# dropbox/rust-brotli

Hardware: AMD Instinct MI355X
Metric: compress MB/s at q5 lgwin22 (higher is better)
Workload: dtype u8; 1 GPU; 64 MiB synthetic English-like text per GPU, quality=5, lgwin=22, one-shot BrotliEncoderCompress (H6), input and stream resident in HBM; input_bytes_total=67108864, compressed_bytes=16370400

## Files before the change

rust-brotli_amd/csrc/device_api.h:

```cpp
#ifndef BROTLI_MI355X_DEVICE_API_H_
#define BROTLI_MI355X_DEVICE_API_H_

#include <stddef.h>
#include <stdint.h>

#include <vector>

#include "lz77_types.h"

#define BR_STREAM (::brotli_mi355x::dev_stream_flushed())

struct ihipStream_t;
namespace brotli_mi355x {

ihipStream_t* dev_stream_flushed();

void* dev_alloc(size_t bytes);
void* dev_alloc_uninit(size_t bytes);
#ifdef BROTLI_HOST_EMU
void dev_free(void* p);
#else
void dev_free(void* p) noexcept;
static_assert(noexcept(dev_free(nullptr)), "blocks are freed in destructors");
#endif
void dev_memset(void* p, int value, size_t bytes);
void dev_h2d(void* dst, const void* src, size_t bytes);
void dev_d2h(void* dst, const void* src, size_t bytes);
void dev_h2d_bulk(void* dst, const void* src, size_t bytes);
void dev_d2h_bulk(void* dst, const void* src, size_t bytes);
void dev_d2h_async(void* dst, const void* src, size_t bytes);
void dev_d2d(void* dst, const void* src, size_t bytes);
void dev_sync();
void dev_mark();
void dev_wait_mark();
void dev_mark_n(int i);
void dev_wait_mark_n(int i);
void* dev_host_alloc(size_t bytes);
void dev_host_free(void* p);
void dev_pool_counters(double* out4, bool reset);
void dev_make_room_for(size_t bytes, size_t own_share);
void dev_make_room(unsigned min_free_share);
size_t dev_trim_pool();
int dev_current_device();
void dev_use_device(int device);
int dev_device_count();
const char* dev_name();

class DevBlocks {
 public:
  DevBlocks() = default;
  DevBlocks(DevBlocks&& o) noexcept : blocks_(std::move(o.blocks_)) { o.blocks_.clear(); }
  DevBlocks& operator=(DevBlocks&& o) noexcept {
    if (this != &o) {
      clear();
      blocks_.swap(o.blocks_);
    }
    return *this;
  }
  ~DevBlocks() { clear(); }
  template <typename T = void>
  T* zeroed(size_t bytes) { return (T*)get(bytes, true); }
  template <typename T = void>
  T* uninit(size_t bytes) { return (T*)get(bytes, false); }
  template <typename T>
  void drop(T*& p) {
    if (p) dev_free(forget(p));
    p = nullptr;
  }
  template <typename T>
  T* give(DevBlocks& to, T*& p) {
    T* q = p;
    to.blocks_.reserve(to.blocks_.size() + 1);
    to.blocks_.push_back(forget(p));
    p = nullptr;
    return q;
  }
  void clear() noexcept {
    for (void* p : blocks_) dev_free(p);
    blocks_.clear();
  }

 private:
  void* get(size_t bytes, bool zero) {
    blocks_.reserve(blocks_.size() + 1);
    blocks_.push_back(zero ? dev_alloc(bytes) : dev_alloc_uninit(bytes));
    return blocks_.back();
  }
  void* forget(const void* p) {
    for (size_t i = blocks_.size(); i-- > 0;)
      if (blocks_[i] == p) {
        void* q = blocks_[i];
        blocks_.erase(blocks_.begin() + (ptrdiff_t)i);
        return q;
      }
    return nullptr;
  }
  std::vector<void*> blocks_;
};

struct DevMem {
  DevBlocks blocks;
  static constexpr size_t kArenaBytes = (size_t)4 << 20, kSmall = (size_t)256 << 10;
  uint8_t* arena = nullptr;
  size_t arena_used = kArenaBytes;
  template <typename T>
  T* alloc(size_t count) {
    const size_t bytes = (count * sizeof(T) + 64 + 255) & ~(size_t)255;
    if (bytes > kSmall) return blocks.zeroed<T>(bytes);
    if (arena_used + bytes > kArenaBytes) {
      arena = blocks.zeroed<uint8_t>(kArenaBytes);
      arena_used = 0;
    }
    T* p = (T*)(arena + arena_used);
    arena_used += bytes;
    return p;
  }
};

struct DeviceTables {
  const uint16_t* dict_hash;
  const uint8_t* dict_data;
  const uint32_t* dict_offsets_by_length;
  const uint8_t* dict_size_bits_by_length;
  const float* logs_16;
  const float* logs_8;
  const uint8_t* utf8_context_lookup;
  const uint8_t* signed_context_lookup;
  const uint16_t* dict_lut_buckets;
  const uint32_t* dict_lut_words;
};
const DeviceTables& dev_tables();

static constexpr uint32_t kChangedCap = 1u << 16;
struct RankInitialHint {
  uint32_t first_block_start, block_bytes;
  uint32_t prefix_is_dictionary;
};
struct SegGeometry;

struct Lz77Buffers {
  uint8_t* text;
  uint16_t* keys;
  uint32_t* by_key;
  uint16_t* sorted_keys;
  uint8_t* fbits;
  uint32_t* info[2];
  uint32_t* sorted[2];
  uint32_t* key_base;
  uint32_t* key_first;
  uint32_t* key_last;
  uint32_t* changed_keys;
  uint32_t* changed_count;
  uint16_t* stag;
  uint32_t* rows;
  void* checkpoints = nullptr;
  uint32_t* rows_changed_lo = nullptr;
  uint32_t* rows_changed_hi = nullptr;
  uint32_t splice_lists = 1;
  uint32_t* dict_items = nullptr;
  uint32_t* changed_slot;
  uint32_t* row_ctl;
  uint32_t* reset_counts;
  const uint32_t* count_base;
  uint32_t* run_end;
  unsigned long long* smask;
  uint32_t* gprev;
  uint8_t* big_tile;
  unsigned long long* pot = nullptr;
  uint32_t* pot_state = nullptr;
  uint32_t* pot_list = nullptr;
  uint32_t pot_list_cap = 0;
  uint32_t* flip_cells = nullptr;
  uint32_t cell_shift = 0, cells_per_key = 0;
  uint32_t changed_cap;
  uint16_t* sorted_tag[2] = {nullptr, nullptr};
  uint32_t* search_log = nullptr;
  uint32_t* recheck_list = nullptr;
  uint32_t* recheck_count = nullptr;
  uint32_t recheck_cap = 0;
  uint8_t* flags[2];
  Command* cmds;
  Segment* segments;
  SegEntry* entries;
  SegExit* exits;
  void* sort_tmp;
  size_t sort_tmp_bytes;
};

size_t lz77_sort_tmp_bytes(uint32_t total_bytes);

void lz77_compute_keys(const Lz77Params& P, const Lz77Buffers& B);
void lz77_run_table(const Lz77Params& P, const Lz77Buffers& B);
void lz77_init_flags(const Lz77Params& P, const Lz77Buffers& B, uint32_t first_block_start, const uint8_t* prefix_flags_host = nullptr,
                     uint32_t prefix_flags_bytes = 0);
void lz77_sort_by_key(const Lz77Params& P, const Lz77Buffers& B);
void lz77_rank_flags(const Lz77Params& P, const Lz77Buffers& B, int which, int rbuf, const RankInitialHint* initial = nullptr);
void lz77_rows_init(const Lz77Params& P, const Lz77Buffers& B, int which, const RankInitialHint* initial, bool has_big_keys);
void lz77_rows_update(const Lz77Params& P, const Lz77Buffers& B, int prev, int next, const SegGeometry& geo, uint8_t* dirty_dev,
                      bool has_big_keys);
void lz77_parse_round(const Lz77Params& P, const Lz77Buffers& B, int which, int rbuf, uint32_t first_segment);
void lz77_parse_list(const Lz77Params& P, const Lz77Buffers& B, int which, int rbuf, const uint32_t* list_dev, uint8_t* sched_dev,
                     uint32_t count);
void lz77_scatter_entries(const Lz77Buffers& B, const uint32_t* index_dev, const SegEntry* entries_dev, uint32_t count);
void lz77_gather_results(const Lz77Buffers& B, const uint32_t* list_dev, uint32_t count, const uint8_t* sched_dev, uint32_t num_segments,
                         SegExit* exits_out, uint32_t* cont_count, uint32_t* cont_index, SegExit* cont_exits, SegEntry* cont_entries);
void lz77_diff_flags(const Lz77Params& P, const Lz77Buffers& B, int prev, int next);
struct BurstBuffers {
  uint8_t* sched = nullptr;
  uint8_t* cand_dirty = nullptr;
  uint8_t* entry_dirty = nullptr;
  uint8_t* touched = nullptr;
  uint8_t* stale = nullptr;
  SegEntry* new_entries = nullptr;
  uint32_t* list = nullptr;
  uint32_t* counters = nullptr;
};
void lz77_chain_check(const Lz77Params& P, const Lz77Buffers& B, const BurstBuffers& U);
void lz77_flags_catch_up(const Lz77Params& P, const Lz77Buffers& B, const BurstBuffers& U, int src, int dst);
void lz77_diff_flags_touched(const Lz77Params& P, const Lz77Buffers& B, const BurstBuffers& U, int prev, int next);
void lz77_reset_rows_changed(const Lz77Params& P, const Lz77Buffers& B);
void lz77_drop_checkpoints(const Lz77Params& P, const Lz77Buffers& B, const uint32_t* list_dev, uint32_t count);
void lz77_burst_count(const Lz77Params& P, const Lz77Buffers& B, const BurstBuffers& U);
void lz77_burst_schedule(const Lz77Params& P, const Lz77Buffers& B, const BurstBuffers& U);
void lz77_gather_touched(const Lz77Params& P, const Lz77Buffers& B, const BurstBuffers& U, uint32_t* index_out, SegExit* exits_out, SegEntry* entries_out);
struct SegGeometry {
  uint32_t prefix_bytes, first_block_start, block_bytes, num_blocks, num_segments, block_size ;
  const uint32_t* block_first_segment;
  const uint32_t* block_segment_bytes;
};
void lz77_validate(const Lz77Params& P, const Lz77Buffers& B, int which, int rbuf_old, int rbuf_new, const SegGeometry& geo,
                   uint8_t* dirty_dev);
void lz77_recheck_searches(const Lz77Params& P, const Lz77Buffers& B, int rbuf, const SegGeometry& geo, uint8_t* dirty_dev);
static constexpr uint32_t kRerankChunk = 4096;
struct RerankChunk {
  uint32_t key_lo;
  uint32_t begin, end;
  uint32_t first_sum;
  uint32_t my_sum;
};
void lz77_rerank_keys(const Lz77Params& P, const Lz77Buffers& B, int which, int rbuf, const RerankChunk* chunks_dev, uint32_t num_chunks,
                      uint32_t* sums_dev, const SegGeometry& geo, uint8_t* dirty_dev);
void lz77_parse_custom(const Lz77Params& P, const Lz77Buffers& B, int which, int rbuf, const Segment* segments_dev,
                       SegEntry* entries_dev, SegExit* exits_dev, uint32_t count);
struct CacheCheck {
  uint32_t segment;
  int32_t cache[4];
};
void lz77_check_cache(const Lz77Params& P, const Lz77Buffers& B, int which, const CacheCheck* items_dev, uint32_t count, uint8_t* ok_dev);
void lz77_key_counts(const Lz77Params& P, const Lz77Buffers& B, int which, uint32_t upto, uint32_t* out_dev, bool with_base = true);
void lz77_parse_timing(double* total_ms, uint32_t* launches, uint64_t* segments, uint64_t* work = nullptr);
void lz77_sample_histograms(const uint8_t* text_dev, const uint32_t* ranges, uint32_t count, uint32_t* out);
void lz77_sample_histogram(const uint8_t* text, uint32_t start, uint32_t bytes, uint32_t* histo256_dev);
void lz77_gather_commands(const Lz77Params& P, const Lz77Buffers& B, uint32_t num_segments, const uint32_t* offsets_dev,
                          const uint32_t* counts_dev, Command* out);

struct ZopfliJob {
  uint32_t quality = 10, lgwin = 22;
  uint32_t use_dictionary = 1;
  uint32_t dist_alphabet_size = 0;
  uint32_t block_bytes = 0;
  uint32_t* buckets = nullptr;
  uint32_t* forest = nullptr;
  void* nodes = nullptr;
  float* literal_costs = nullptr;
  float* cost_dist = nullptr;
  float* cost_cmd = nullptr;
  unsigned long long* matches = nullptr;
  uint32_t* num_matches = nullptr;
  Command* tmp_cmds = nullptr;
  uint32_t* histo = nullptr;
  uint32_t* forest_new = nullptr;
  uint32_t* forest_bak = nullptr;
  uint32_t* buckets_bak = nullptr;
  uint8_t* rerooted = nullptr;
  uint32_t* ctl = nullptr;
};
void lz77_zopfli_init(const ZopfliJob& J);
void lz77_zopfli_import(const ZopfliJob& J, const uint32_t* buckets_src, const uint32_t* forest_src, uint32_t delta);
void lz77_zopfli_prepend(const Lz77Params& P, const Lz77Buffers& B, const ZopfliJob& J, uint32_t dict_bytes);
bool lz77_zopfli_block(const Lz77Params& P, const Lz77Buffers& B, const ZopfliJob& J, uint32_t block);

struct LiveBuffers {
  uint16_t* num = nullptr;
  uint32_t* buckets = nullptr;
  uint32_t* slot_of = nullptr;
  uint32_t* rank[2] = {nullptr, nullptr};
  uint32_t* entry[2] = {nullptr, nullptr};
  uint8_t* changed_key = nullptr;
  LiveBlockState* state = nullptr;
  uint32_t tables = 0;
  uint32_t span_blocks = 1;
};
void lz77_live_slots(const Lz77Params& P, const Lz77Buffers& B, const LiveBuffers& L);
void lz77_live_index(const Lz77Params& P, const Lz77Buffers& B, const LiveBuffers& L, int which);
void lz77_live_materialise(const Lz77Params& P, const Lz77Buffers& B, const LiveBuffers& L, int which, const uint32_t* first_dev,
                           const uint32_t* start_dev, uint32_t count);
void lz77_live_parse(const Lz77Params& P, const Lz77Buffers& B, const LiveBuffers& L, int which, const uint32_t* first_dev, uint32_t count);
void lz77_live_verify(const Lz77Params& P, const Lz77Buffers& B, const LiveBuffers& L, int prev, int next, const SegGeometry& geo,
                      const uint8_t* reparsed_dev, uint8_t* dirty_dev);

void lz77_patch_commands(Command* cmds, const CmdPatch* patches_dev, uint32_t n);

template <typename T>
struct PinnedArray {
  T* ptr = nullptr;
  size_t cap = 0, n = 0;
  PinnedArray() = default;
  PinnedArray(const PinnedArray&) = delete;
  PinnedArray& operator=(const PinnedArray&) = delete;
  ~PinnedArray() { dev_host_free(ptr); }
  void resize_discard(size_t count) {
    if (count > cap) {
      dev_host_free(ptr);
      cap = count + count / 4 + 16;
      ptr = (T*)dev_host_alloc(cap * sizeof(T));
    }
    n = count;
  }
  void assign(size_t count, const T& v) {
    resize_discard(count);
    for (size_t i = 0; i < count; ++i) ptr[i] = v;
  }
  T* data() { return ptr; }
  const T* data() const { return ptr; }
  size_t size() const { return n; }
  T& operator[](size_t i) { return ptr[i]; }
  const T& operator[](size_t i) const { return ptr[i]; }
};

}
#endif
```

rust-brotli_amd/csrc/lz77_kernels.hip:

```cpp
#include <hip/hip_runtime.h>
#include <stdexcept>
#include <string>
#include <utility>
#include <string.h>
#include <mutex>
#include <vector>

#include "device_api.h"
#include "lz77_chain.h"
#include "lz77_rows.h"
#include "lz77_groups.h"
#include "device_scan.h"
#include "lz77_parse_args.h"
#include "zopfli_device.h"
#include "batch_greedy_device.h"

namespace brotli_mi355x {

void hip_check(hipError_t e, const char* what) {
  if (e == hipSuccess) return;
  (void)hipGetLastError();
  throw std::runtime_error(std::string("HIP error in ") + what + ": " + hipGetErrorString(e));
}

static constexpr uint32_t kSortTile = 4096;

__global__ __launch_bounds__(256) void k_compute_keys(const uint8_t* __restrict__ text, uint16_t* __restrict__ keys,
                                                      uint32_t n, uint32_t valid_n, uint32_t kind, uint32_t bucket_bits,
                                                      uint64_t hash_mask, uint32_t* __restrict__ run_samples,
                                                      const uint16_t* __restrict__ dict_hash, uint32_t* __restrict__ dict_items,
                                                      uint32_t num_tiles, uint32_t* __restrict__ hist) {
  __shared__ uint32_t h[256];
  for (uint32_t tile = blockIdx.x; tile < num_tiles; tile += gridDim.x) {
    const uint32_t tile_base = tile * kSortTile;
    const uint32_t tile_n = n - tile_base < kSortTile ? n - tile_base : kSortTile;
    if (hist != nullptr) {
      h[threadIdx.x] = 0;
      __syncthreads();
    }
#pragma unroll 4
    for (uint32_t e = threadIdx.x; e < tile_n; e += 256) {
      const uint32_t i = tile_base + e;
      if (dict_items != nullptr) {
        const uint32_t dh = ((br_load32(text + i) * 0x1e35a7bdu) >> (32 - 14)) << 1;
        dict_items[i] = (uint32_t)dict_hash[dh] | ((uint32_t)dict_hash[dh + 1] << 16);
      }
      uint32_t key = 0xffffu;
      if (i < valid_n) {
        if ((i & 63u) == 0 && i + 16 <= n) {
          const uint64_t v = br_load64(text + i);
          if (v == (v & 0xffull) * 0x0101010101010101ull && br_load64(text + i + 8) == v && *(volatile uint32_t*)run_samples < 4096u)
            atomicAdd(run_samples, 1u);
        }
        if (kind == 6) {
          const uint64_t v = (br_load64(text + i) & hash_mask) * 0x1fe35a7bd3579bd3ull;
          key = (uint32_t)(v >> (64 - bucket_bits));
        } else {
          const uint32_t v = br_load32(text + i) * 0x1e35a7bdu;
          key = v >> (32 - bucket_bits);
        }
      }
      keys[i] = (uint16_t)key;
      if (hist != nullptr) atomicAdd(&h[key & 255u], 1u);
    }
    if (hist != nullptr) {
      __syncthreads();
      hist[threadIdx.x * num_tiles + tile] = h[threadIdx.x];
    }
  }
  if (dict_items != nullptr && blockIdx.x == 0 && threadIdx.x == 0) {
    const uint32_t dh = ((br_load32(text + n) * 0x1e35a7bdu) >> (32 - 14)) << 1;
    dict_items[n] = (uint32_t)dict_hash[dh] | ((uint32_t)dict_hash[dh + 1] << 16);
  }
}

struct SortScratch {
  uint16_t* keys_tmp;
  uint32_t* vals_tmp;
  uint16_t* tags_tmp;
  uint32_t* hist;
  uint32_t* scratch;
};
static SortScratch sort_scratch(const Lz77Buffers& B, uint32_t n) {
  const uint32_t tiles = (n + kSortTile - 1) / kSortTile;
  SortScratch s;
  uint8_t* tmp = (uint8_t*)B.sort_tmp;
  s.keys_tmp = (uint16_t*)tmp;
  tmp += ((size_t)n * 2 + 255) & ~(size_t)255;
  s.vals_tmp = (uint32_t*)tmp;
  tmp += ((size_t)n * 4 + 255) & ~(size_t)255;
  s.tags_tmp = (uint16_t*)tmp;
  tmp += ((size_t)n * 2 + 255) & ~(size_t)255;
  s.hist = (uint32_t*)tmp;
  tmp += (size_t)tiles * 256 * 4;
  s.scratch = (uint32_t*)tmp;
  return s;
}

void lz77_compute_keys(const Lz77Params& P, const Lz77Buffers& B) {
  const uint32_t n = P.total_bytes;
  const uint32_t valid_n = n >= P.htl ? n - P.htl + 1 : 0;
  const uint64_t hash_mask = P.hasher_kind == 6 ? (0xffffffffffffffffull >> (64 - 8 * P.hash_len)) : 0;
  if (n == 0) return;
  const uint32_t tiles = (n + kSortTile - 1) / kSortTile;
  uint32_t* hist = (B.sort_tmp != nullptr && B.sort_tmp_bytes >= lz77_sort_tmp_bytes(n)) ? sort_scratch(B, n).hist : nullptr;
  dev_memset(B.changed_count + 8, 0, 4);
  hipLaunchKernelGGL(k_compute_keys, dim3(tiles < 8192 ? tiles : 8192), dim3(256), 0, BR_STREAM, B.text, B.keys, n, valid_n, P.hasher_kind,
                     P.bucket_bits, hash_mask, B.changed_count + 8, dev_tables().dict_hash, B.dict_items, tiles, hist);
  HIP_CHECK(hipGetLastError());
}

__global__ __launch_bounds__(64) void k_init_flag_tails(const Segment* __restrict__ segments, uint32_t num_segments, uint32_t htl,
                                                         uint8_t* __restrict__ flags) {
  const uint32_t k = blockIdx.x * blockDim.x + threadIdx.x;
  if (k >= num_segments) return;
  const Segment g = segments[k];
  if (!(g.flags & kSegFirstInBlock)) return;
  const uint32_t bs = g.blk_start, be = g.blk_end;
  if (g.block_index == 0 && be - bs >= htl - 1 && bs >= 3) flags[bs - 3] = flags[bs - 2] = flags[bs - 1] = 1;
  const uint32_t store_end = (be - bs >= htl) ? be - htl + 1 : bs;
  for (uint32_t q = store_end; q < be; ++q) flags[q] = (q + 3 >= be && (g.flags & kSegTailStitched)) ? 1 : 0;
}

void lz77_init_flags(const Lz77Params& P, const Lz77Buffers& B, uint32_t first_block_start, const uint8_t* prefix_flags_host,
                     uint32_t prefix_flags_bytes) {
  const uint32_t M = P.total_bytes, P0 = P.prefix_bytes, htl = P.htl;
  dev_memset(B.flags[0], 0, (size_t)M + 64);
  if (P0 > htl - 1) HIP_CHECK(hipMemsetAsync(B.flags[0], 1, P0 - (htl - 1), BR_STREAM));
  if (prefix_flags_host && prefix_flags_bytes) {
    HIP_CHECK(hipMemcpyAsync(B.flags[0], prefix_flags_host, prefix_flags_bytes, hipMemcpyHostToDevice, BR_STREAM));
  }
  if (M > first_block_start) HIP_CHECK(hipMemsetAsync(B.flags[0] + first_block_start, 1, M - first_block_start, BR_STREAM));
  if (P.num_segments) {
    hipLaunchKernelGGL(k_init_flag_tails, dim3((P.num_segments + 63) / 64), dim3(64), 0, BR_STREAM, B.segments, P.num_segments, htl, B.flags[0]);
  }
  HIP_CHECK(hipMemcpyAsync(B.flags[1], B.flags[0], (size_t)M + 64, hipMemcpyDeviceToDevice, BR_STREAM));
  HIP_CHECK(hipGetLastError());
}

__global__ __launch_bounds__(256) void k_radix_hist(const uint16_t* __restrict__ keys, uint32_t n, uint32_t shift,
                                                     uint32_t num_tiles, uint32_t* __restrict__ hist) {
  __shared__ uint32_t h[256];
  h[threadIdx.x] = 0;
  __syncthreads();
  const uint32_t base = blockIdx.x * kSortTile;
  for (uint32_t r = 0; r < 16; ++r) {
    const uint32_t i = base + r * 256 + threadIdx.x;
    if (i < n) atomicAdd(&h[(keys[i] >> shift) & 255u], 1u);
  }
  __syncthreads();
  hist[threadIdx.x * num_tiles + blockIdx.x] = h[threadIdx.x];
}

template <bool kFirstPass>
__global__ __launch_bounds__(256) __attribute__((amdgpu_waves_per_eu(4, 4))) void k_radix_scatter(const uint16_t* __restrict__ keys_in, const uint32_t* __restrict__ vals_in,
                                                        uint16_t* __restrict__ keys_out, uint32_t* __restrict__ vals_out, uint32_t n,
                                                        uint32_t shift, uint32_t num_tiles, const uint32_t* __restrict__ offsets,
                                                        const uint8_t* __restrict__ text, const uint16_t* __restrict__ tags_in,
                                                        uint16_t* __restrict__ tags_out, uint32_t* __restrict__ key_first,
                                                        uint32_t* __restrict__ key_last) {
  __shared__ uint32_t gbase[256];
  __shared__ uint32_t lstart[257];
  __shared__ uint32_t wbase[4][256];
  __shared__ uint32_t wave_total[4];
  __shared__ uint16_t skey[kSortTile];
  __shared__ uint32_t sval[kSortTile];
  __shared__ uint16_t stagv[kSortTile];
  const int tid = threadIdx.x, lane = tid & 63, w = tid >> 6;
  const uint32_t tile_base = blockIdx.x * kSortTile;
  const uint32_t tile_n = n - tile_base < kSortTile ? n - tile_base : kSortTile;
  const uint32_t hidx = (uint32_t)tid * num_tiles + blockIdx.x;
  const uint32_t here = offsets[hidx];
  const uint32_t next = hidx + 1 < 256u * num_tiles ? offsets[hidx + 1] : n;
  uint32_t key[16], val[16], tag[16];
  const uint32_t e0 = (uint32_t)w * 1024u + (uint32_t)lane;
#pragma unroll
  for (int r = 0; r < 16; ++r) {
    const uint32_t e = e0 + (uint32_t)r * 64u;
    key[r] = keys_in[tile_base + (e < tile_n ? e : tile_n - 1)];
  }
#pragma unroll
  for (int r = 0; r < 16; ++r) {
    const uint32_t e = e0 + (uint32_t)r * 64u;
    const uint32_t i = tile_base + (e < tile_n ? e : tile_n - 1);
    val[r] = kFirstPass ? i : vals_in[i];
  }
  if (tags_out != nullptr) {
#pragma unroll
    for (int r = 0; r < 16; ++r) {
      const uint32_t e = e0 + (uint32_t)r * 64u;
      const uint32_t i = tile_base + (e < tile_n ? e : tile_n - 1);
      tag[r] = kFirstPass ? br_tag16(br_load32(text + i)) : (uint32_t)tags_in[i];
    }
  }
  const uint32_t count = next - here;
  uint32_t start;
  {
    gbase[tid] = here;
    uint32_t incl = count;
    for (uint32_t o = 1; o < 64; o <<= 1) {
      const uint32_t up = (uint32_t)__shfl_up((int)incl, o, 64);
      if ((uint32_t)lane >= o) incl += up;
    }
    if (lane == 63) wave_total[w] = incl;
#pragma unroll
    for (int j = 0; j < 4; ++j) wbase[w][lane * 4 + j] = 0;
    __syncthreads();
    uint32_t before = 0;
    for (int i = 0; i < w; ++i) before += wave_total[i];
    start = before + incl - count;
    lstart[tid] = start;
    if (tid == 255) lstart[256] = start + count;
  }
  volatile uint32_t* mine = wbase[w];
#pragma unroll
  for (int r = 0; r < 16; ++r) {
    const bool valid = e0 + (uint32_t)r * 64u < tile_n;
    const uint32_t d = (key[r] >> shift) & 255u;
    unsigned long long peers = __ballot(valid);
#pragma unroll
    for (int bit = 0; bit < 8; ++bit) {
      const bool one = (d >> bit) & 1u;
      const unsigned long long b = __ballot(one);
      peers &= one ? b : ~b;
    }
    const uint32_t rank_in_wave = __popcll(peers & ((1ull << lane) - 1ull));
    const uint32_t seen = mine[d];
    key[r] |= (seen + rank_in_wave) << 16;
    __builtin_amdgcn_wave_barrier();
    if (valid && rank_in_wave == 0) mine[d] = seen + (uint32_t)__popcll(peers);
    __builtin_amdgcn_wave_barrier();
  }
  __syncthreads();
  {
    const uint32_t c0 = wbase[0][tid], c1 = wbase[1][tid], c2 = wbase[2][tid];
    wbase[0][tid] = start;
    wbase[1][tid] = start + c0;
    wbase[2][tid] = start + c0 + c1;
    wbase[3][tid] = start + c0 + c1 + c2;
  }
  __syncthreads();
#pragma unroll
  for (int r = 0; r < 16; ++r) {
    if (e0 + (uint32_t)r * 64u < tile_n) {
      const uint32_t at = wbase[w][(key[r] >> shift) & 255u] + (key[r] >> 16);
      skey[at] = (uint16_t)key[r];
      sval[at] = val[r];
      if (tags_out != nullptr) stagv[at] = (uint16_t)tag[r];
    }
  }
  __syncthreads();
  for (uint32_t at = tid; at < tile_n; at += 256) {
    const uint32_t k = skey[at];
    const uint32_t d = (k >> shift) & 255u;
    const uint32_t ls = lstart[d];
    const uint32_t dst = gbase[d] + (at - ls);
    keys_out[dst] = (uint16_t)k;
    vals_out[dst] = sval[at];
    if (tags_out != nullptr) tags_out[dst] = stagv[at];
    if (!kFirstPass && key_first != nullptr) {
// ... 1153 lines not shown
    P.masked_from = kNeverMasked;
    P.htl = kSpec;
    br_parse_chain<kH9, kRows, kSplice>(P, a.T, scratch, a.segments, a.entries, a.exits, k, a.sched, a.max_continuation);
  } else {
    br_parse_chain<kH9, kRows, kSplice>(a.P, a.T, scratch, a.segments, a.entries, a.exits, k, a.sched, a.max_continuation);
  }
}

#if !defined(BR_GROUP_WAVES)
#define BR_GROUP_WAVES 3
#endif
template <uint32_t kHtl>
__global__ __launch_bounds__(64) __attribute__((amdgpu_waves_per_eu(BR_GROUP_WAVES, BR_GROUP_WAVES))) void k_parse_groups(ParseArgs a) {
  __shared__ uint32_t dict_off[32];
  if (threadIdx.x < 32) dict_off[threadIdx.x] = threadIdx.x < 25 ? a.T.dict_offsets_by_length[threadIdx.x] : 0u;
  __builtin_amdgcn_wave_barrier();
  uint32_t item = blockIdx.x;
  if (a.per_xcd) item = (blockIdx.x & 7u) * a.per_xcd + (blockIdx.x >> 3);
  const uint32_t i = item * 4u + (threadIdx.x >> 4);
  const bool have = i < a.count;
  const uint32_t k = a.first_segment + (have ? i : 0u);
  Lz77Params P = a.P;
  P.ndist = 4;
  P.block_bits = 4;
  P.spree_window = 64;
  P.score_per_byte = 135;
  P.dict_break = 0;
  P.reset_pos = 0;
  P.masked_from = kNeverMasked;
  P.htl = kHtl;
  uint32_t walked, searches, commands;
  br_group_parse<kHtl>(P, a.T, a.segments[k], a.entries[k], a.exits[k], have, dict_off, &walked, &searches, &commands);
  if (a.T.work && have && (threadIdx.x & 15u) == 0) {
    atomicAdd(a.T.work + 0, (unsigned long long)walked);
    atomicAdd(a.T.work + 1, (unsigned long long)searches);
    atomicAdd(a.T.work + 2, (unsigned long long)commands);
  }
}

static void launch_parse(const Lz77Params& P, const Lz77Buffers& B, int flags_in, int flags_out, int rbuf, const Segment* segments,
                         SegEntry* entries, SegExit* exits, uint32_t first_segment, const uint32_t* list, uint8_t* sched,
                         uint32_t count) {
  const DeviceTables& dt = dev_tables();
  ParseArgs a;
  a.P = P;
  a.T.text = B.text;
  a.T.info = B.info[rbuf];
  a.T.sorted = B.sorted[rbuf];
  a.T.sorted_tag = (!B.rows && B.stag) ? B.sorted_tag[rbuf] : nullptr;
  a.T.rows = B.rows;
  a.T.dict_items = B.dict_items;
  a.T.run_end = B.run_end;
  a.T.search_log = B.rows ? nullptr : B.search_log;
  a.T.flags_next = B.flags[flags_out];
  a.T.cmds = B.cmds;
  a.T.dict_hash = dt.dict_hash;
  a.T.dict_data = dt.dict_data;
  a.T.dict_offsets_by_length = dt.dict_offsets_by_length;
  a.T.dict_size_bits_by_length = dt.dict_size_bits_by_length;
  a.T.dist_postfix_bits = P.dist_postfix_bits;
  a.T.num_direct_distance_codes = P.num_direct_distance_codes;
  {
    ParseTiming& ptw = parse_timing();
    if (!ptw.work_dev) {
      HIP_CHECK(hipMalloc((void**)&ptw.work_dev, 4 * sizeof(unsigned long long)));
      dev_memset(ptw.work_dev, 0, 4 * sizeof(unsigned long long));
    }
    a.T.work = ptw.work_dev;
  }
  a.segments = segments;
  a.entries = entries;
  a.exits = exits;
  a.first_segment = first_segment;
  a.list = list;
  a.sched = sched;
  static const uint32_t tuned = getenv("BROTLI_MI355X_CONT") ? (uint32_t)atoi(getenv("BROTLI_MI355X_CONT")) : kMaxContinuation;
  a.max_continuation = count <= 256 ? 1024u : tuned;
  a.count = count;
  ParseTiming& pt = parse_timing();
  if (pt.used == pt.events.size()) {
    hipEvent_t n0, n1;
    HIP_CHECK(hipEventCreate(&n0));
    HIP_CHECK(hipEventCreate(&n1));
    pt.events.push_back(std::make_pair(n0, n1));
  }
  const hipEvent_t e0 = pt.events[pt.used].first, e1 = pt.events[pt.used].second;
  pt.used++;
  HIP_CHECK(hipEventRecord(e0, BR_STREAM));
  static const bool xcd_aware = getenv("BROTLI_MI355X_NO_XCD_MAP") == nullptr;
  a.per_xcd = (xcd_aware && count >= 64) ? (count + 7) / 8 : 0;
  const uint32_t grid = a.per_xcd ? a.per_xcd * 8 : count;
  static const uint32_t lds_pad = getenv("BROTLI_MI355X_LDS_PAD") ? (uint32_t)atoi(getenv("BROTLI_MI355X_LDS_PAD")) : 0u;
  static const uint32_t groups_min = getenv("BROTLI_MI355X_GROUPS_MIN") ? (uint32_t)atoi(getenv("BROTLI_MI355X_GROUPS_MIN")) : 0xffffffffu;
  const bool groups = B.rows && list == nullptr && sched == nullptr && count >= groups_min && plain_q5_config(P) && getenv("BROTLI_MI355X_NO_SPEC") == nullptr;
  if (groups) {
    const bool own = segments == B.segments;
    a.T.checkpoints = own ? (Checkpoint*)B.checkpoints : nullptr;
    const uint32_t waves = (count + 3u) / 4u;
    a.per_xcd = (xcd_aware && waves >= 64) ? (waves + 7) / 8 : 0;
    const uint32_t ggrid = a.per_xcd ? a.per_xcd * 8 : waves;
    if (P.htl == 8) hipLaunchKernelGGL((k_parse_groups<8>), dim3(ggrid), dim3(64), 0, BR_STREAM, a);
    else hipLaunchKernelGGL((k_parse_groups<4>), dim3(ggrid), dim3(64), 0, BR_STREAM, a);
  } else if (P.hasher_kind == 9) {
    hipLaunchKernelGGL((k_parse_segments<true, false>), dim3(grid), dim3(64), lds_pad, BR_STREAM, a);
  } else if (B.rows) {
    static const bool spec_off = getenv("BROTLI_MI355X_NO_SPEC") != nullptr;
    static const bool splice_off = getenv("BROTLI_MI355X_NO_SPLICE") != nullptr;
    const uint32_t spec = (!spec_off && plain_q5_config(P)) ? P.htl : 0u;
    const bool own_segments = segments == B.segments;
    a.T.checkpoints = own_segments ? (Checkpoint*)B.checkpoints : nullptr;
    a.T.rows_changed_lo = B.rows_changed_lo;
    a.T.rows_changed_hi = B.rows_changed_hi;
    static const uint32_t splice_part_off = getenv("BROTLI_MI355X_SPLICE_OFF") ? (uint32_t)atoi(getenv("BROTLI_MI355X_SPLICE_OFF")) : 0u;
    a.T.splice_off = splice_part_off;
    const bool splice = !splice_off && sched != nullptr && own_segments && B.checkpoints != nullptr && B.splice_lists != 0;
    if (spec == 8) {
      if (splice) hipLaunchKernelGGL((k_parse_segments<false, true, 8, true>), dim3(grid), dim3(64), lds_pad, BR_STREAM, a);
      else hipLaunchKernelGGL((k_parse_segments<false, true, 8>), dim3(grid), dim3(64), lds_pad, BR_STREAM, a);
    } else if (spec == 4) {
      if (splice) hipLaunchKernelGGL((k_parse_segments<false, true, 4, true>), dim3(grid), dim3(64), lds_pad, BR_STREAM, a);
      else hipLaunchKernelGGL((k_parse_segments<false, true, 4>), dim3(grid), dim3(64), lds_pad, BR_STREAM, a);
    } else {
      if (splice) hipLaunchKernelGGL((k_parse_segments<false, true, 0, true>), dim3(grid), dim3(64), lds_pad, BR_STREAM, a);
      else hipLaunchKernelGGL((k_parse_segments<false, true>), dim3(grid), dim3(64), lds_pad, BR_STREAM, a);
    }
  } else if (P.block_bits > 7) {
    hipLaunchKernelGGL((k_parse_segments<false, false, 0, false, true>), dim3(grid), dim3(64), lds_pad, BR_STREAM, a);
  } else {
    hipLaunchKernelGGL((k_parse_segments<false, false>), dim3(grid), dim3(64), lds_pad, BR_STREAM, a);
  }
  HIP_CHECK(hipEventRecord(e1, BR_STREAM));
  HIP_CHECK(hipGetLastError());
  pt.counts.push_back(count);
  pt.segments += count;
}

void lz77_parse_round(const Lz77Params& P, const Lz77Buffers& B, int which, int rbuf, uint32_t first_segment) {
  if (first_segment >= P.num_segments) return;
  launch_parse(P, B, which, which ^ 1, rbuf, B.segments, B.entries, B.exits, first_segment, nullptr, nullptr, P.num_segments - first_segment);
}

void lz77_parse_list(const Lz77Params& P, const Lz77Buffers& B, int which, int rbuf, const uint32_t* list_dev, uint8_t* sched_dev,
                     uint32_t count) {
  if (count == 0) return;
  launch_parse(P, B, which, which ^ 1, rbuf, B.segments, B.entries, B.exits, 0, list_dev, sched_dev, count);
}

void lz77_parse_custom(const Lz77Params& P, const Lz77Buffers& B, int which, int rbuf, const Segment* segments_dev,
                       SegEntry* entries_dev, SegExit* exits_dev, uint32_t count) {
  if (count == 0) return;
  launch_parse(P, B, which, which ^ 1, rbuf, segments_dev, entries_dev, exits_dev, 0, nullptr, nullptr, count);
}

struct FlipCells {
  uint32_t* bits;
  uint32_t shift, per_key, words;
};
__device__ __forceinline__ void mark_flip_cell(const FlipCells& c, uint32_t key, uint32_t pos) {
  const uint32_t cell = key * c.per_key + (pos >> c.shift);
  const uint32_t bit = 1u << (cell & 31u);
  if (!(c.bits[cell >> 5] & bit)) atomicOr(&c.bits[cell >> 5], bit);
}
static FlipCells flip_cells_of(const Lz77Buffers& B) {
  FlipCells c;
  c.bits = B.rows ? B.flip_cells : nullptr;
  c.shift = B.cell_shift;
  c.per_key = B.cells_per_key;
  c.words = (uint32_t)(((size_t)65536 * B.cells_per_key) / 32);
  return c;
}
static void clear_flip_cells(const Lz77Buffers& B) {
  if (B.rows && B.flip_cells) dev_memset(B.flip_cells, 0, ((size_t)65536 * B.cells_per_key) / 8 + 8);
}

__global__ __launch_bounds__(256) void k_diff_flags(const uint8_t* __restrict__ prev, const uint8_t* __restrict__ next, uint32_t n,
                                                     const uint16_t* __restrict__ keys, uint32_t* __restrict__ changed_keys,
                                                     uint32_t* __restrict__ changed_count, uint32_t cap, uint32_t emit_positions, FlipCells cells) {
  const uint32_t words = (n + 15) / 16;
  const uint32_t lane = threadIdx.x & 63u;
  for (uint32_t w0 = (blockIdx.x * blockDim.x + threadIdx.x) - lane; w0 < words; w0 += gridDim.x * blockDim.x) {
    const uint32_t wi = w0 + lane;
    uint32_t d[4] = {0, 0, 0, 0};
    if (wi < words) {
      const uint4 a = ((const uint4*)prev)[wi], b = ((const uint4*)next)[wi];
      d[0] = (a.x ^ b.x) & 0x05050505u;
      d[1] = (a.y ^ b.y) & 0x05050505u;
      d[2] = (a.z ^ b.z) & 0x05050505u;
      d[3] = (a.w ^ b.w) & 0x05050505u;
      for (uint32_t j = 0; j < 4; ++j) d[j] = (d[j] | (d[j] >> 2)) & 0x01010101u;
      for (uint32_t j = 0; j < 16; ++j)
        if (wi * 16 + j >= n) d[j >> 2] &= ~(1u << (8 * (j & 3)));
    }
    const uint32_t mine = (uint32_t)(__popc(d[0]) + __popc(d[1]) + __popc(d[2]) + __popc(d[3]));
    if (__ballot(mine != 0) == 0) continue;
    uint32_t incl = mine;
    for (uint32_t off = 1; off < 64; off <<= 1) {
      const uint32_t up = (uint32_t)__shfl_up((int)incl, off, 64);
      if (lane >= off) incl += up;
    }
    uint32_t base = 0;
    uint32_t sat = 0;
    if (lane == 63) {
      if (*(volatile const uint32_t*)changed_count > cap) {
        base = cap;
        sat = 1;
        if (cells.bits) cells.bits[cells.words] = 1;
      } else {
        base = atomicAdd(changed_count, incl);
      }
    }
    base = (uint32_t)__shfl((int)base, 63, 64);
    sat = (uint32_t)__shfl((int)sat, 63, 64);
    uint32_t idx = base + incl - mine;
    const bool mark = cells.bits != nullptr && sat == 0;
    if (mine == 0 || (idx >= cap && !mark)) continue;
    for (uint32_t j = 0; j < 16; ++j) {
      if ((d[j >> 2] >> (8 * (j & 3))) & 1u) {
        if (idx < cap) changed_keys[idx] = emit_positions ? wi * 16 + j : (uint32_t)keys[wi * 16 + j];
        if (mark) mark_flip_cell(cells, keys[wi * 16 + j], wi * 16 + j);
        ++idx;
      }
    }
  }
}

__global__ __launch_bounds__(256) void k_scatter_entries(SegEntry* __restrict__ entries, const uint32_t* __restrict__ index,
                                                          const SegEntry* __restrict__ src, uint32_t count) {
  const uint32_t t = blockIdx.x * blockDim.x + threadIdx.x;
  if (t >= count * 16u) return;
  ((uint32_t*)(entries + index[t >> 4]))[t & 15u] = ((const uint32_t*)src)[t];
}

void lz77_scatter_entries(const Lz77Buffers& B, const uint32_t* index_dev, const SegEntry* entries_dev, uint32_t count) {
  static_assert(sizeof(SegEntry) == 64, "k_scatter_entries copies 16 words per entry");
  if (count == 0) return;
  hipLaunchKernelGGL(k_scatter_entries, dim3((count * 16u + 255) / 256), dim3(256), 0, BR_STREAM, B.entries, index_dev, entries_dev, count);
  HIP_CHECK(hipGetLastError());
}

__global__ __launch_bounds__(256) void k_gather_results(const SegExit* __restrict__ exits, const SegEntry* __restrict__ entries,
                                                         const uint32_t* __restrict__ list, uint32_t count, const uint8_t* __restrict__ sched,
                                                         uint32_t num_segments, SegExit* __restrict__ exits_out, uint32_t* __restrict__ cont_count,
                                                         uint32_t* __restrict__ cont_index, SegExit* __restrict__ cont_exits,
                                                         SegEntry* __restrict__ cont_entries) {
  const uint32_t t = blockIdx.x * blockDim.x + threadIdx.x;
  if (t < count) exits_out[t] = exits[list[t]];
  if (t < num_segments && sched[t] == 3) {
    const uint32_t j = atomicAdd(cont_count, 1u);
    cont_index[j] = t;
    cont_exits[j] = exits[t];
    cont_entries[j] = entries[t];
  }
}

void lz77_gather_results(const Lz77Buffers& B, const uint32_t* list_dev, uint32_t count, const uint8_t* sched_dev, uint32_t num_segments,
                         SegExit* exits_out, uint32_t* cont_count, uint32_t* cont_index, SegExit* cont_exits, SegEntry* cont_entries) {
  dev_memset(cont_count, 0, 4);
  const uint32_t n = count > num_segments ? count : num_segments;
  hipLaunchKernelGGL(k_gather_results, dim3((n + 255) / 256), dim3(256), 0, BR_STREAM, B.exits, B.entries, list_dev, count, sched_dev, num_segments,
                     exits_out, cont_count, cont_index, cont_exits, cont_entries);
  HIP_CHECK(hipGetLastError());
}

__global__ __launch_bounds__(256) void k_chain_check(const Segment* __restrict__ segments, const SegEntry* __restrict__ entries,
                                                      const SegExit* __restrict__ exits, uint32_t num_segments, const uint8_t* __restrict__ sched,
                                                      uint8_t* __restrict__ touched, uint8_t* __restrict__ entry_dirty, SegEntry* __restrict__ new_entries,
                                                      uint32_t* __restrict__ rows_lo, uint32_t* __restrict__ rows_hi, uint8_t* __restrict__ stale) {
  const uint32_t k = blockIdx.x * blockDim.x + threadIdx.x;
  if (k < num_segments) br_chain_check(segments, entries, exits, num_segments, k, sched, touched, entry_dirty, new_entries, rows_lo, rows_hi, stale);
}
void lz77_chain_check(const Lz77Params& P, const Lz77Buffers& B, const BurstBuffers& U) {
  hipLaunchKernelGGL(k_chain_check, dim3((P.num_segments + 255) / 256), dim3(256), 0, BR_STREAM, B.segments, B.entries, B.exits, P.num_segments,
                     U.sched, U.touched, U.entry_dirty, U.new_entries, B.rows_changed_lo, B.rows_changed_hi, U.stale);
  HIP_CHECK(hipGetLastError());
}

__global__ __launch_bounds__(64) void k_flags_catch_up(const Segment* __restrict__ segments, uint32_t num_segments, uint8_t* __restrict__ stale,
                                                        const uint8_t* __restrict__ src, uint8_t* __restrict__ dst) {
  const uint32_t k = blockIdx.x;
  if (k >= num_segments || !stale[k]) return;
  const uint32_t a = segments[k].start, b = segments[k].end;
  const uint32_t wa = (a + 15u) / 16u, wb = b / 16u;
  if (wa < wb) {
    for (uint32_t w = wa + threadIdx.x; w < wb; w += 64) ((uint4*)dst)[w] = ((const uint4*)src)[w];
    for (uint32_t q = a + threadIdx.x; q < wa * 16u; q += 64) dst[q] = src[q];
    for (uint32_t q = wb * 16u + threadIdx.x; q < b; q += 64) dst[q] = src[q];
  } else {
    for (uint32_t q = a + threadIdx.x; q < b; q += 64) dst[q] = src[q];
  }
  if (threadIdx.x == 0) stale[k] = 0;
}
void lz77_flags_catch_up(const Lz77Params& P, const Lz77Buffers& B, const BurstBuffers& U, int src, int dst) {
  if (P.num_segments == 0) return;
  hipLaunchKernelGGL(k_flags_catch_up, dim3(P.num_segments), dim3(64), 0, BR_STREAM, B.segments, P.num_segments, U.stale, B.flags[src], B.flags[dst]);
  HIP_CHECK(hipGetLastError());
}

__global__ __launch_bounds__(64) void k_diff_flags_touched(const Segment* __restrict__ segments, uint32_t num_segments, const uint8_t* __restrict__ stale,
                                                            const uint8_t* __restrict__ prev, const uint8_t* __restrict__ next,
                                                            uint32_t* __restrict__ changed_pos, uint32_t* __restrict__ changed_count, uint32_t cap,
                                                            const uint16_t* __restrict__ keys, FlipCells cells) {
  const uint32_t k = blockIdx.x;
  if (k >= num_segments || !stale[k]) return;
  const uint32_t a = segments[k].start, b = segments[k].end;
  const uint32_t lane = threadIdx.x;
  for (uint32_t w0 = a / 16u; w0 * 16u < b; w0 += 64) {
// ... 1086 lines not shown
```

rust-brotli_amd/csrc/lz77_stage.cpp:

```cpp
#include "lz77_stage.h"
#include "timeline.h"

#include <math.h>
#include <stdio.h>
#include <stdlib.h>
#include <string.h>

#include <algorithm>
#include <chrono>
#include <map>
#include <stdexcept>
#include <string>

#include "host_entropy.h"

#include <cmath>

namespace brotli_mi355x {

void Lz77Stage::Release() {
  mem_.clear();
  L_ = LiveBuffers{};
  Z_ = ZopfliJob{};
  S_ = QuickSpec{};
  Q_ = QuickJob{};
  count_base_dev_ = qsnap_table_ = zsnap_buckets_ = zsnap_forest_ = nullptr;
  histo_dev_ = gather_offsets_dev_ = gather_counts_dev_ = nullptr;
  gathered_cmds_ = nullptr;
  gathered_capacity_ = 0;
}

void Lz77Stage::SetupCommon(bool with_sort_tmp) {
  cmds_bytes_ = (size_t)total_cmd_slots_ * sizeof(Command) + 64;
  B_.cmds = mem_.uninit<Command>(cmds_bytes_);
  B_.segments = mem_.zeroed<Segment>(segments_.size() * sizeof(Segment) + 64);
  B_.entries = mem_.zeroed<SegEntry>(segments_.size() * sizeof(SegEntry) + 64);
  B_.exits = mem_.zeroed<SegExit>(segments_.size() * sizeof(SegExit) + 64);
  if (with_sort_tmp) {
    B_.sort_tmp_bytes = lz77_sort_tmp_bytes(P_.total_bytes);
    B_.sort_tmp = mem_.uninit(B_.sort_tmp_bytes);
  }
  histo_dev_ = mem_.zeroed<uint32_t>(256 * 4);
  gather_offsets_dev_ = mem_.zeroed<uint32_t>(segments_.size() * 4 + 64);
  gather_counts_dev_ = mem_.zeroed<uint32_t>(segments_.size() * 4 + 64);
  segments_upload_.resize_discard(segments_.size());
  memcpy(segments_upload_.data(), segments_.data(), segments_.size() * sizeof(Segment));
  dev_h2d(B_.segments, segments_upload_.data(), segments_.size() * sizeof(Segment));
}

void Lz77Stage::Setup(const EncoderParams& params, uint8_t* text_dev, uint32_t prefix_bytes, uint32_t input_bytes,
                      uint32_t raw_head_bytes, uint32_t segment_bytes) {
  Release();
  coarse_blocks_.clear();
  params_ = params;
  input_bytes_ = input_bytes;
  raw_head_bytes_ = raw_head_bytes;
  block_bytes_ = 1u << params.lgblock;
  segment_bytes_ = std::min(std::max(segment_bytes, 256u), block_bytes_);
  memset(&P_, 0, sizeof(P_));
  P_.total_bytes = prefix_bytes + input_bytes;
  P_.prefix_bytes = prefix_bytes;
  P_.dict_break = (carry_ && carry_->valid) ? carry_->dict_break : prefix_bytes;
  P_.ring_mask = (1u << ComputeRbBits(params)) - 1u;
  P_.max_backward_limit = (1u << params.lgwin) - 16u;
  P_.hasher_kind = params.hasher.type == 5 ? 5 : (params.hasher.type == 9 ? 9 : 6);
  P_.bucket_bits = (uint32_t)params.hasher.bucket_bits;
  P_.block_bits = (uint32_t)params.hasher.block_bits;
  P_.hash_len = (uint32_t)params.hasher.hash_len;
  P_.ndist = (uint32_t)params.hasher.num_last_distances_to_check;
  P_.htl = P_.hasher_kind == 6 ? 8 : 4;
  P_.literal_byte_score = (uint32_t)(params.hasher.literal_byte_score ? params.hasher.literal_byte_score : 540);
  P_.score_per_byte = P_.literal_byte_score >> 2;
  P_.use_dictionary = params.use_dictionary ? 1 : 0;
  P_.spree_window = params.quality < 9 ? 64 : 512;
  P_.dist_max_distance = (uint32_t)params.dist.max_distance;
  P_.quality = (uint32_t)params.quality;
  P_.dist_postfix_bits = params.dist.distance_postfix_bits;
  P_.num_direct_distance_codes = params.dist.num_direct_distance_codes;
  P_.cmd_slab_stride = segment_bytes_ / 2 + 8;
  P_.block_bytes = block_bytes_;
  P_.max_metablock_bytes = (uint32_t)MaxMetablockSize(params);
  BuildSegments();
  P_.num_segments = (uint32_t)segments_.size();

  const size_t M = P_.total_bytes;
  B_ = Lz77Buffers{};
  B_.text = text_dev;
  use_zopfli_ = params.hasher.type == 10;
  use_quick_ = params.hasher.type == 2 || params.hasher.type == 3 || params.hasher.type == 4 || params.hasher.type == 54;
  if (use_quick_) {
    use_live_ = use_rows_ = false;
    P_.htl = 8;
    use_qspec_ = getenv("BROTLI_MI355X_QUICK_SERIAL") == nullptr && input_bytes >= 64 && (uint64_t)P_.total_bytes * 2 < 0xfffffff0ull;
    qspec_books_in_ = false;
    qspec_coarse_ = false;
    qspec_params_ = params;
    qspec_text_ = text_dev;
    qspec_prefix_ = prefix_bytes;
    qspec_input_ = input_bytes;
    qspec_raw_head_ = raw_head_bytes;
    if (!use_qspec_ && segment_bytes_ != block_bytes_) segment_bytes_ = block_bytes_;
    P_.cmd_slab_stride = segment_bytes_ / 2 + 8;
    BuildSegments();
    P_.num_segments = (uint32_t)segments_.size();
    Q_ = QuickJob{};
    Q_.kind = (uint32_t)params.hasher.type;
    Q_.bucket_bits = Q_.kind == 54 ? 20 : (Q_.kind == 4 ? 17 : 16);
    Q_.sweep = Q_.kind == 2 ? 1 : (Q_.kind == 3 ? 2 : 4);
    Q_.hash_len = Q_.kind == 54 ? 7 : 5;
    Q_.use_dictionary = (params.use_dictionary && (Q_.kind == 2 || Q_.kind == 4)) ? 1 : 0;
    P_.use_dictionary = use_qspec_ ? Q_.use_dictionary : 0;
    Q_.table = mem_.uninit<uint32_t>((size_t)quick_table_words(Q_) * 4 + 64);
    if (use_qspec_) {
      S_ = QuickSpec{};
      S_.n = P_.total_bytes;
      S_.events = Q_.sweep == 1 ? S_.n : 2u * S_.n;
      S_.slots = quick_slots(Q_);
      const size_t E = S_.events, N = S_.n;
      S_.ev_slot = mem_.uninit<uint32_t>(E * 4 + 64);
      S_.ev_id = mem_.uninit<uint32_t>(E * 4 + 64);
      S_.ev_of = mem_.uninit<uint32_t>(E * 4 + 64);
      S_.slot_first = mem_.uninit<uint32_t>(((size_t)S_.slots + 2) * 4 + 64);
      S_.qrank = mem_.uninit<uint32_t>(N * Q_.sweep * 4 + 64);
      S_.actraw = mem_.uninit<uint32_t>(E * 4 + 64);
      S_.act = mem_.uninit<uint32_t>(E * 4 + 64);
      S_.val = mem_.uninit<uint32_t>(E * 4 + 64);
      S_.cand = mem_.uninit<uint32_t>(N * Q_.sweep * 4 + 64);
      S_.flags = mem_.uninit<uint8_t>(N + 64);
      S_.flags_prev = mem_.uninit<uint8_t>(N + 64);
      S_.chg_cap = (uint32_t)std::max<size_t>(4096, E / (getenv("BROTLI_MI355X_QUICK_CAP_DIV") ? (size_t)atoi(getenv("BROTLI_MI355X_QUICK_CAP_DIV")) : 16));
      S_.chg_list = mem_.uninit<uint32_t>((size_t)S_.chg_cap * 4 + 64);
      S_.chg_range = mem_.uninit<uint32_t>((size_t)S_.chg_cap * 12 + 64);
      S_.chg_count = mem_.zeroed<uint32_t>(64);
      S_.sort_tmp_bytes = lz77_qspec_sort_tmp_bytes(S_.events);
      S_.sort_tmp = mem_.uninit(S_.sort_tmp_bytes);
      S_.sort_keys_tmp = mem_.uninit<uint32_t>(E * 4 + 64);
      S_.sort_ids_tmp = mem_.uninit<uint32_t>(E * 4 + 64);
      S_.scan_tmp = mem_.uninit<uint32_t>((E / 1024 + E / (1024 * 1024) + 8192) * 4);
    }
    SetupCommon(false);
    exits_.assign((uint32_t)segments_.size(), SegExit{});
    return;
  }
  if (use_zopfli_) {
    use_live_ = use_rows_ = false;
    if (segment_bytes_ != block_bytes_) {
      segment_bytes_ = block_bytes_;
      P_.cmd_slab_stride = segment_bytes_ / 2 + 8;
      BuildSegments();
      P_.num_segments = (uint32_t)segments_.size();
    }
    P_.use_dictionary = 0;
    P_.hasher_kind = 5;
    P_.bucket_bits = 16;
    P_.htl = 4;
    B_.keys = mem_.uninit<uint16_t>(M * 2 + 64);
    B_.by_key = mem_.uninit<uint32_t>(M * 4 + 64);
    B_.sorted_keys = mem_.uninit<uint16_t>(M * 2 + 64);
    B_.key_first = mem_.zeroed<uint32_t>((65536 + 1) * 4);
    B_.key_last = mem_.zeroed<uint32_t>((65536 + 1) * 4);
    B_.changed_count = mem_.zeroed<uint32_t>(64);
    B_.sort_tmp_bytes = lz77_sort_tmp_bytes(P_.total_bytes);
    B_.sort_tmp = mem_.uninit(B_.sort_tmp_bytes);
    Z_ = ZopfliJob{};
    Z_.quality = (uint32_t)params.quality;
    Z_.lgwin = (uint32_t)params.lgwin;
    Z_.use_dictionary = params.use_dictionary ? 1 : 0;
    Z_.dist_alphabet_size = params.dist.alphabet_size;
    Z_.block_bytes = block_bytes_;
// ... 31 lines not shown
    const uint64_t base = (carry_ && carry_->valid) ? carry_->stream_base : 0;
    if (base >= ring) P_.masked_from = 0;
    else if (base + P_.total_bytes > ring) P_.masked_from = (uint32_t)(ring - base);
  }
  use_live_ = P_.hasher_kind != 9 && (P_.masked_from != kNeverMasked || getenv("BROTLI_MI355X_LIVE") != nullptr);
  if (use_live_) {
    use_rows_ = false;
    if (segment_bytes_ != block_bytes_) {
      segment_bytes_ = block_bytes_;
      P_.cmd_slab_stride = segment_bytes_ / 2 + 8;
      BuildSegments();
      P_.num_segments = (uint32_t)segments_.size();
    }
    const size_t K = (size_t)1 << P_.bucket_bits;
    L_.span_blocks = (uint32_t)std::max<size_t>(1, segments_.size());
    L_.tables = 1;
    L_.num = mem_.uninit<uint16_t>(K * 2 + 64);
    L_.buckets = mem_.uninit<uint32_t>((K << P_.block_bits) * 4 + 64);
    L_.state = mem_.zeroed<LiveBlockState>(segments_.size() * sizeof(LiveBlockState) + 64);
    live_verify_ = getenv("BROTLI_MI355X_LIVE_VERIFY") != nullptr || getenv("BROTLI_MI355X_SELFTEST") != nullptr;
    L_.slot_of = mem_.uninit<uint32_t>(M * 4 + 64);
    for (int i = 0; i < 2; ++i) {
      L_.rank[i] = mem_.uninit<uint32_t>((M + 1) * 4 + 64);
      L_.entry[i] = mem_.uninit<uint32_t>(M * 4 + 64);
    }
    if (live_verify_) {
      B_.search_log = mem_.zeroed<uint32_t>(M * kSearchLogWords * 4 + 64);
      B_.recheck_cap = (uint32_t)(M + 4096);
      B_.recheck_list = mem_.uninit<uint32_t>((size_t)B_.recheck_cap * 4 + 64);
      B_.recheck_count = mem_.zeroed<uint32_t>(64);
    }
    L_.changed_key = mem_.zeroed<uint8_t>(65536 + 64);
    B_.changed_cap = kChangedCap;
    B_.changed_keys = mem_.zeroed<uint32_t>((size_t)kChangedCap * 4);
  } else
  if (use_rows_) {
    B_.changed_cap = (uint32_t)std::max<size_t>(kChangedCap, M / 32);
    B_.changed_keys = mem_.uninit<uint32_t>((size_t)B_.changed_cap * 4 + 64);
    B_.changed_slot = mem_.uninit<uint32_t>((size_t)B_.changed_cap * 4 + 64);
    B_.row_ctl = mem_.zeroed<uint32_t>(64);
    B_.big_tile = mem_.zeroed<uint8_t>(M / 1024 + 128);
    B_.smask = mem_.uninit<unsigned long long>((M / 64 + 2) * 8 + 64);
    B_.gprev = mem_.uninit<uint32_t>((M / 64 + 2) * 4 + 64);
    if (getenv("BROTLI_MI355X_NO_POTENTIAL_MASK") == nullptr) {
      B_.pot = mem_.uninit<unsigned long long>((M / 64 + 2) * 8 + 64);
      B_.pot_state = mem_.zeroed<uint32_t>(64);
      B_.pot_list_cap = (uint32_t)(M / 16 + 1024);
      B_.pot_list = mem_.uninit<uint32_t>((size_t)B_.pot_list_cap * 4 + 64);
      if (getenv("BROTLI_MI355X_NO_FLIP_CELLS") == nullptr) {
        uint32_t shift = 8;
        while (shift < 31 && (1u << shift) < P_.max_backward_limit + 1u) ++shift;
        while (shift < 31 && (M >> shift) + 2 > 1024) ++shift;
        B_.cell_shift = shift;
        B_.cells_per_key = (uint32_t)(M >> shift) + 2;
        B_.flip_cells = mem_.zeroed<uint32_t>((size_t)65536 * B_.cells_per_key / 8 + 64);
      }
    }
    B_.stag = mem_.uninit<uint16_t>(M * 2 + 64);
    B_.rows = mem_.uninit<uint32_t>(M * kRowEntries * 4 + 64);
    if (P_.use_dictionary) B_.dict_items = mem_.uninit<uint32_t>(M * 4 + 256);
    if (getenv("BROTLI_MI355X_NO_CHECKPOINTS") == nullptr) {
      B_.checkpoints = mem_.zeroed((M / kCheckpointStride + 2) * sizeof(Checkpoint));
      B_.rows_changed_lo = mem_.uninit<uint32_t>(segments_.size() * 4 + 64);
      B_.rows_changed_hi = mem_.uninit<uint32_t>(segments_.size() * 4 + 64);
    }
  } else {
    B_.changed_cap = kChangedCap;
    B_.changed_keys = mem_.zeroed<uint32_t>((size_t)kChangedCap * 4);
    B_.info[0] = mem_.uninit<uint32_t>(M * 8 + 64);
    B_.info[1] = mem_.uninit<uint32_t>(M * 8 + 64);
    B_.sorted[0] = mem_.zeroed<uint32_t>(M * 4 + 64);
    B_.sorted[1] = mem_.zeroed<uint32_t>(M * 4 + 64);
    if (getenv("BROTLI_MI355X_NO_TAGS") == nullptr) {
      B_.stag = mem_.uninit<uint16_t>(M * 2 + 64);
      B_.sorted_tag[0] = mem_.zeroed<uint16_t>(M * 2 + 64);
      B_.sorted_tag[1] = mem_.zeroed<uint16_t>(M * 2 + 64);
    }
    if (getenv("BROTLI_MI355X_NO_RECHECK") == nullptr) {
      B_.search_log = mem_.zeroed<uint32_t>(M * kSearchLogWords * 4 + 64);
      B_.recheck_cap = (uint32_t)std::max<size_t>(4096, M / 8);
      B_.recheck_list = mem_.uninit<uint32_t>((size_t)B_.recheck_cap * 4 + 64);
      B_.recheck_count = mem_.zeroed<uint32_t>(64);
    }
  }
  B_.key_base = mem_.zeroed<uint32_t>((65536 + 1) * 4);
  B_.reset_counts = mem_.zeroed<uint32_t>((65536 + 1) * 4);
  B_.flags[0] = mem_.zeroed<uint8_t>(M + 64);
  B_.flags[1] = mem_.zeroed<uint8_t>(M + 64);
  SetupCommon(true);
}

void Lz77Stage::BuildSegments() {
  segments_.clear();
  const uint32_t P0 = P_.prefix_bytes;
  const uint32_t end = P_.total_bytes;
  const uint32_t htl = P_.htl;
  std::vector<std::pair<uint32_t, uint32_t>> blocks;
  for (uint64_t off = 0; off < input_bytes_; off += block_bytes_) {
    uint32_t bs = P0 + (uint32_t)off;
    uint32_t be = (uint32_t)std::min<uint64_t>(end, (uint64_t)P0 + off + block_bytes_);
    if (off == 0) bs = std::min(be, bs + raw_head_bytes_);
    blocks.emplace_back(bs, be);
  }
  uint32_t cmd_base = 0;
  block_first_segment_.clear();
  block_segment_bytes_.clear();
  for (size_t b = 0; b < blocks.size(); ++b) {
    const uint32_t bs = blocks[b].first, be = blocks[b].second;
    bool stitched = false;
    if (b + 1 < blocks.size()) {
      const uint32_t nbytes = blocks[b + 1].second - blocks[b + 1].first;
      stitched = nbytes >= htl - 1 && blocks[b + 1].first >= 3;
    }
    const uint32_t seg_bytes = (b < coarse_blocks_.size() && coarse_blocks_[b]) ? block_bytes_ : segment_bytes_;
    block_first_segment_.push_back((uint32_t)segments_.size());
    block_segment_bytes_.push_back(seg_bytes);
    uint32_t s = bs;
    bool first = true;
    do {
      const uint32_t e = std::min(be, s + seg_bytes);
      Segment g;
      g.start = s;
      g.end = e;
      g.blk_start = bs;
      g.blk_end = be;
      g.flags = (first ? kSegFirstInBlock : 0u) | (e == be ? kSegLastInBlock : 0u) | (stitched ? kSegTailStitched : 0u);
      g.cmd_base = cmd_base;
      g.block_index = (uint32_t)b;
      g.cmd_cap = (e - s) / 2 + 8;
      cmd_base += g.cmd_cap;
      segments_.push_back(g);
      first = false;
      s = e;
    } while (s < be);
  }
  block_first_segment_.push_back((uint32_t)segments_.size());
  total_cmd_slots_ = cmd_base;
}

void Lz77Stage::InitFlags() {
  const bool cont = carry_ && carry_->valid;
  lz77_init_flags(P_, B_, segments_.empty() ? P_.total_bytes : segments_[0].blk_start, cont ? carry_->stored.data() : nullptr,
                  cont ? (uint32_t)std::min<size_t>(carry_->stored.size(), P_.prefix_bytes) : 0u);
}

struct DictTracker {
  enum State { kAlive, kFuzzy, kDead, kUnknown };
  bool use = false;
  State state = kAlive;
  uint32_t L = 0, M = 0;
  int64_t slack = 0;
  uint32_t left_alive_at = 0xffffffffu;
  uint32_t flips = 0;
  static constexpr uint32_t kDeadL = 0x40000000u, kDeadM = 0;
  static constexpr uint32_t kAliveL = 0, kAliveM = 0x01000000u;
  static constexpr int64_t kSlackPerChain = 256;
  void Hint(SegEntry* e) const {
    switch (state) {
      case kAlive:
        e->dict_lookups = L;
        e->dict_matches = M;
        e->dict_exact = 1;
        break;
      case kFuzzy:
        e->dict_lookups = kAliveL;
        e->dict_matches = kAliveM;
        e->dict_exact = 0;
        break;
      default:
        e->dict_lookups = kDeadL;
        e->dict_matches = kDeadM;
        e->dict_exact = state == kDead;
        break;
    }
  }
  bool Consume(uint32_t k, const SegEntry& used, const SegExit& x) {
    if (!use) return true;
    if (state == kAlive && M < (L >> 7)) {
      state = kDead;
      left_alive_at = k;
    }
    const bool no_match = x.dict_matches == used.dict_matches;
    if (state == kDead || state == kUnknown) {
      const bool ok = x.dict_mode == 0 || x.dict_mode == 2 || x.dict_mode == 4 || (x.dict_mode == 1 && no_match);
      if (!ok) flips++;
      return ok;
    }
    const bool exact = state == kAlive && used.dict_lookups == L && used.dict_matches == M;
    const bool stays_alive = 128ll * (int64_t)M - (int64_t)L + 127 - slack >= (int64_t)x.dict_maxdef;
    bool ok = true;
    State next = state;
    switch (x.dict_mode) {
      case 0:
        break;
      case 4:
        ok = false;
        next = kFuzzy;
        slack += kSlackPerChain;
        break;
      case 1:
        if (exact || stays_alive) {
          L += x.dict_lookups - used.dict_lookups;
          M += x.dict_matches - used.dict_matches;
        } else if (no_match) {
          next = state == kAlive ? kDead : kUnknown;
        } else {
          ok = false;
          next = kUnknown;
        }
        break;
      case 2:
        if (no_match) {
          if (stays_alive) {
            L += x.dict_lookups - used.dict_lookups;
          } else {
            next = state == kAlive ? kDead : kUnknown;
          }
        } else {
          ok = false;
          next = kFuzzy;
          slack += kSlackPerChain;
        }
        break;
      default:
        if (exact) {
          next = kDead;
        } else {
          ok = false;
          next = kUnknown;
        }
        break;
    }
    if ((!ok || next != state) && getenv("BROTLI_MI355X_DEBUG_DICT"))
      fprintf(stderr, "  dict seg %u: state %d->%d L %u M %u slack %lld used (%u,%u,%u) exit (%u,%u) mode %u maxdef %d ok %d\n", k, (int)state,
              (int)next, L, M, (long long)slack, used.dict_lookups, used.dict_matches, used.dict_exact, x.dict_lookups, x.dict_matches,
              x.dict_mode, x.dict_maxdef, (int)ok);
    if (next != state) {
      if (next == kDead || next == kUnknown) left_alive_at = k;
      state = next;
    }
    return ok;
  }
};

static void PredictLiteralRunStepwise(const Lz77Params& P, const Segment& seg, const SegEntry& e, SegExit* x) {
  const uint32_t pos_end = seg.blk_end, htl = P.htl, window = P.spree_window;
  const uint32_t margin = htl - 1 > 4 ? htl - 1 : 4;
  uint32_t position = e.pos;
  const uint32_t apply = e.apply;
  uint32_t tail_kind = e.head_kind, tail_base = e.head_base;
  const uint32_t tail_p1 = e.head_p1;
  while (position + htl < pos_end && position < seg.end) {
    position++;
    if (position > apply) {
      if (position + 16 >= pos_end - margin) {
        tail_kind = kHeadUnstored;
        tail_base = position;
        position = pos_end;
      } else if (position > apply + 4 * window) {
        tail_kind = kHeadVec4;
        tail_base = position;
        position += 16;
      } else {
        tail_kind = kHeadEven4;
        tail_base = position;
        position += 8;
      }
    }
  }
  if (seg.flags & kSegLastInBlock) position = pos_end;
  x->pos = position;
  x->apply = apply;
  x->insert_len = position - e.pos;
  x->tail_kind = position > seg.end ? tail_kind : (uint32_t)kHeadNone;
  x->tail_base = position > seg.end ? tail_base : 0u;
  x->tail_p1 = position > seg.end ? tail_p1 : 0u;
}

static void PredictLiteralRun(const Lz77Params& P, const Segment& seg, const SegEntry& e, SegExit* x) {
  const uint64_t pos_end = seg.blk_end, htl = P.htl, window = P.spree_window;
  const uint64_t margin = htl - 1 > 4 ? htl - 1 : 4;
  uint64_t position = e.pos;
  const uint64_t apply = e.apply;
  uint32_t tail_kind = e.head_kind;
  uint64_t tail_base = e.head_base;
  const uint64_t stop = std::min<uint64_t>(pos_end > htl ? pos_end - htl : 0, seg.end);
  if (position < stop && position < apply) position = std::min(stop, apply);
  const uint64_t block_tail = pos_end > margin + 16 ? pos_end - margin - 16 : 0;
  auto stride = [&](uint64_t step, uint64_t p_limit, uint32_t kind) {
    uint64_t bound = stop;
    bound = std::min(bound, block_tail > 0 ? block_tail - 1 : 0);
    bound = std::min(bound, p_limit);
    if (position >= bound) return;
    const uint64_t n = (bound - position + step - 1) / step;
    tail_kind = kind;
    tail_base = position + (n - 1) * step + 1;
    position += n * step;
  };
  if (position < stop) stride(9, apply + 4 * window, kHeadEven4);
  if (position < stop && position + 1 > apply + 4 * window) stride(17, ~0ull >> 1, kHeadVec4);
  if (position < stop && position + 1 >= block_tail && position + 1 > apply) {
    tail_kind = kHeadUnstored;
    tail_base = position + 1;
    position = pos_end;
  }
  if (seg.flags & kSegLastInBlock) position = pos_end;
  x->pos = (uint32_t)position;
  x->apply = (uint32_t)apply;
  x->insert_len = (uint32_t)position - e.pos;
  x->tail_kind = position > seg.end ? tail_kind : (uint32_t)kHeadNone;
  x->tail_base = position > seg.end ? (uint32_t)tail_base : 0u;
  x->tail_p1 = position > seg.end ? e.head_p1 : 0u;
  static const bool selftest = getenv("BROTLI_MI355X_SELFTEST") != nullptr || getenv("BROTLI_MI355X_SELFTEST_RESOLVE") != nullptr;
  if (selftest) {
    SegExit y = *x;
    PredictLiteralRunStepwise(P, seg, e, &y);
    if (y.pos != x->pos || y.apply != x->apply || y.insert_len != x->insert_len || y.tail_kind != x->tail_kind || y.tail_base != x->tail_base ||
        y.tail_p1 != x->tail_p1)
      throw std::runtime_error("selftest: PredictLiteralRun differs from the stepwise loop (segment " + std::to_string(seg.start) + ", entry " +
                               std::to_string(e.pos) + " / " + std::to_string(e.apply) + ")");
  }
}

bool Lz77Stage::FetchShouldCompress() {
  const uint32_t count = (uint32_t)wanted_histograms_.size();
  if (count == 0) return true;
  bool guessed_right = true;
  std::vector<uint32_t> ranges((size_t)count * 2);
  for (uint32_t i = 0; i < count; ++i) {
    ranges[2 * i] = wanted_histograms_[i].first;
    ranges[2 * i + 1] = wanted_histograms_[i].second;
  }
  std::vector<uint32_t> histos((size_t)count * 256);
  lz77_sample_histograms(B_.text, ranges.data(), count, histos.data());
  for (uint32_t i = 0; i < count; ++i) {
    const uint32_t bytes = wanted_histograms_[i].second;
    const float threshold = (float)bytes * 7.92f / 13.0f;
    const bool c = !(HostBitsEntropy(histos.data() + (size_t)i * 256, 256) > threshold);
    should_compress_cache_.emplace(wanted_histograms_[i], c);
    guessed_right = guessed_right && i < wanted_guesses_.size() && (wanted_guesses_[i] != 0) == c;
    if (getenv("BROTLI_MI355X_DEBUG")) fprintf(stderr, "  should_compress sampled [%u,+%u) -> %d\n", wanted_histograms_[i].first, bytes, (int)c);
  }
  wanted_histograms_.clear();
  return guessed_right;
}

bool Lz77Stage::Resolve(bool final_pass) {
  wanted_histograms_.clear();
  wanted_guesses_.clear();
  should_compress_guess_ = true;
  static const bool never_incremental = getenv("BROTLI_MI355X_NO_INCREMENTAL_RESOLVE") != nullptr;
  static const bool check_incremental = getenv("BROTLI_MI355X_SELFTEST") != nullptr || getenv("BROTLI_MI355X_SELFTEST_RESOLVE") != nullptr;
  const bool incremental = resolve_incremental_ && !never_incremental && !use_live_ && block_records_valid_ && !touch_all_;
  resolve_blocks_skipped_ = 0;
  bool consistent = ResolvePass(final_pass, incremental);
  if (!wanted_histograms_.empty()) {
    if (!FetchShouldCompress()) {
      wanted_guesses_.clear();
      should_compress_guess_ = true;
      consistent = ResolvePass(final_pass, false);
      if (!wanted_histograms_.empty()) throw std::runtime_error("brotli_mi355x: the resolver asked for a meta-block twice");
    }
  }
  if (incremental && check_incremental && resolve_blocks_skipped_ != 0) {
    const std::vector<MetaBlockPlan> mb = metablocks_;
    const std::vector<Patch> pa = patches_;
    const std::vector<TrailingInsert> tr = trailing_;
    const std::vector<Carry> ca = carries_;
    const std::vector<SegEntry> ne = next_entries_;
    const std::vector<uint8_t> de = dirty_entry_, er = entry_reason_, pe = predicted_entry_;
    const uint32_t fd = first_dirty_, pr = predicted_runs_, dd = dict_death_seg_, df = dict_flips_, rp = resume_pos_;
    const bool nel = needs_empty_last_;
    const bool full = ResolvePass(final_pass, false);
    auto same_bytes = [](const void* a, const void* b, size_t n) { return n == 0 || memcmp(a, b, n) == 0; };
    const bool same = full == consistent && mb.size() == metablocks_.size() && same_bytes(mb.data(), metablocks_.data(), mb.size() * sizeof(MetaBlockPlan)) &&
                      pa.size() == patches_.size() && same_bytes(pa.data(), patches_.data(), pa.size() * sizeof(Patch)) && tr.size() == trailing_.size() &&
                      same_bytes(tr.data(), trailing_.data(), tr.size() * sizeof(TrailingInsert)) && ca.size() == carries_.size() &&
                      same_bytes(ca.data(), carries_.data(), ca.size() * sizeof(Carry)) && same_bytes(ne.data(), next_entries_.data(), ne.size() * sizeof(SegEntry)) &&
                      de == dirty_entry_ && er == entry_reason_ && pe == predicted_entry_ && fd == first_dirty_ && pr == predicted_runs_ &&
                      dd == dict_death_seg_ && df == dict_flips_ && rp == resume_pos_ && nel == needs_empty_last_;
    if (!same) throw std::runtime_error("selftest: the block-by-block resolver pass differs from the pass over every block");
  }
  touch_all_ = false;
  if (!block_touched_.empty()) std::fill(block_touched_.begin(), block_touched_.end(), (uint8_t)0);
  return consistent;
}

bool Lz77Stage::ResolvePass(bool final_pass, bool incremental) {
  const uint32_t nseg = (uint32_t)segments_.size();
  next_entries_.resize(nseg);
  dbg_mismatch_ = dbg_counts_;
  memset(dbg_counts_, 0, sizeof(dbg_counts_));
  memset(dbg_first_, 0, sizeof(dbg_first_));
  const uint32_t nblocks = (uint32_t)block_segment_bytes_.size();
  if (incremental && (block_records_.size() != (size_t)nblocks + 1 || block_touched_.size() != nblocks || dirty_entry_.size() != nseg)) incremental = false;
  if (incremental) {
    metablocks_prev_.swap(metablocks_);
    trailing_prev_.swap(trailing_);
    carries_prev_.swap(carries_);
  }
  std::vector<ResolveBlockRecord> records((size_t)nblocks + 1);
  metablocks_.clear();
  patches_.clear();
  trailing_.clear();
  carries_.clear();
  bool consistent = true;
  predicted_runs_ = 0;
  first_dirty_ = nseg;
  if (!incremental) {
    dirty_entry_.assign(nseg, 0);
    entry_reason_.assign(nseg, 0);
    predicted_entry_.assign(nseg, 0);
  }
  if (use_live_) live_state_.assign(nseg, LiveBlockState{});
  uint32_t block_marks = 0, block_first_dirty = nseg;
  auto mark = [&](uint32_t k, bool same, uint8_t reason = 1) {
    if (!same) {
      consistent = false;
      dirty_entry_[k] = 1;
      entry_reason_[k] |= reason;
      if (k < first_dirty_) first_dirty_ = k;
      block_marks++;
      if (k < block_first_dirty) block_first_dirty = k;
    }
  };

  int32_t cache[4] = {4, 11, 15, 16};
  if (params_.catable && !params_.catable_behind_init) {
    for (int i = 0; i < 4; ++i) cache[i] = 0x7ffffff0;
  }
  if (carry_ && carry_->valid) memcpy(cache, carry_->dist_cache, sizeof(cache));
  int32_t saved_cache[4];
  memcpy(saved_cache, cache, sizeof(cache));
  uint32_t last_insert_len = 0;
  uint64_t num_commands = 0, num_literals = 0;
  uint32_t last_flush_pos = P_.prefix_bytes + raw_head_bytes_;
  resume_pos_ = last_flush_pos;
  needs_empty_last_ = false;
  DictTracker dict;
  dict.use = P_.use_dictionary != 0;
  if (carry_ && carry_->valid) {
    dict.L = carry_->dict_lookups;
    dict.M = carry_->dict_matches;
    if (carry_->dict_dead) dict.state = DictTracker::kDead;
  }
  if (use_qspec_ && qspec_books_in_) {
    dict.L = qspec_lookups_;
    dict.M = qspec_matches_;
    dict.state = dict.M < (dict.L >> 7) ? DictTracker::kDead : DictTracker::kAlive;
  }
  struct LastCmd {
    bool valid = false;
    uint32_t seg = 0, idx = 0, dist_code = 0, copy_len = 0;
  } last_cmd;
  uint32_t mb_first_seg = 0;
  uint64_t mb_cmds = 0;
  const size_t max_mb = MaxMetablockSize(params_);
  const size_t max_literals = max_mb / 8, max_commands = max_mb / 8;
  (void)final_pass;
  std::map<std::pair<uint32_t, uint32_t>, bool>& should_compress_cache = should_compress_cache_;

  auto flow_now = [&]() {
    ResolveFlow f;
    memset(&f, 0, sizeof(f));
    memcpy(f.cache, cache, sizeof(cache));
// ... 190 lines not shown
      const SegExit& X = *chained;
      int32_t out_cache[4];
      for (uint32_t i = 0; i < 4; ++i) out_cache[i] = i < X.n_pushes ? X.cache[i] : cur_cache[i - X.n_pushes];
      if (substitute_inherited_pushes_ && X.n_pushes != 0 && memcmp(used.cache, cur_cache, sizeof(cur_cache)) != 0) {
        for (uint32_t i = 0; i < 4 && i < X.n_pushes; ++i) {
          int hit = -1;
          bool ambiguous = false;
          for (int c = 0; c < 4; ++c) {
            if (used.cache[c] != out_cache[i]) continue;
            if (hit < 0) hit = c;
            else if (cur_cache[c] != cur_cache[hit]) ambiguous = true;
          }
          if (hit >= 0 && !ambiguous) out_cache[i] = cur_cache[hit];
        }
      }
      if (j == k0 && X.ext_len > 0 && last_cmd.valid) {
        if (!patches_.empty() && patches_.back().segment == last_cmd.seg && patches_.back().index == last_cmd.idx) {
          patches_.back().ext += X.ext_len;
        } else {
          patches_.push_back({last_cmd.seg, last_cmd.idx, X.ext_len});
        }
        records[cur_block].merged_ext = X.ext_len;
        last_cmd.copy_len += X.ext_len;
      }
      num_commands += X.n_cmds;
      mb_cmds += X.n_cmds;
      num_literals += X.n_lits;
      if (X.n_cmds > 0) {
        if (carry != 0) {
          carries_.push_back({j, carry});
          num_literals += carry;
        }
        carry = X.insert_len;
      } else {
        carry += X.insert_len;
      }
      if (X.n_cmds > 0) {
        last_cmd.valid = true;
        last_cmd.seg = j;
        last_cmd.idx = X.n_cmds - 1;
        last_cmd.dist_code = X.last_dist_code;
        last_cmd.copy_len = X.last_copy_len;
      }
      if (j < k1) {
        SegEntry N{};
        N.pos = X.pos;
        N.apply = X.apply;
        memcpy(N.cache, out_cache, sizeof(N.cache));
        N.insert_len = carry;
        N.ext_allowed = 0;
        N.head_kind = X.tail_kind;
        N.head_base = X.tail_base;
        N.head_p1 = X.tail_p1;
        dict.Hint(&N);
        const SegEntry& u = entries_[j + 1];
        const bool cache_same = memcmp(u.cache, N.cache, sizeof(N.cache)) == 0;
        const bool rest_same = u.pos == N.pos && u.apply == N.apply && u.head_kind == N.head_kind && u.head_base == N.head_base && u.head_p1 == N.head_p1;
        if (dbg_mismatch_) {
          dbg_first_[2] += u.head_kind != N.head_kind || u.head_base != N.head_base || u.head_p1 != N.head_p1;
          dbg_mismatch_[0] += u.pos != N.pos;
          dbg_mismatch_[1] += u.pos == N.pos && u.apply != N.apply;
          dbg_mismatch_[2] += u.pos == N.pos && memcmp(u.cache, N.cache, sizeof(N.cache)) != 0;
          dbg_mismatch_[3] += u.pos == N.pos && u.apply != N.apply && memcmp(u.cache, N.cache, sizeof(N.cache)) == 0;
        }
        mark(j + 1, cache_same && rest_same, (uint8_t)((rest_same ? 0 : 1) | (cache_same ? 0 : 2)));
        next_entries_[j + 1] = N;
      }
      memcpy(cur_cache, out_cache, sizeof(cur_cache));
    }
    memcpy(cache, cur_cache, sizeof(cache));
    last_insert_len = carry;
    const bool batch_end = (k1 + 1 == nseg);
    bool is_last = batch_end && !partial_;
    const size_t processed_bytes = be - last_flush_pos;
    const bool should_flush = params_.quality < 4 && num_literals + num_commands >= 0x2fff;
    const bool next_fits = processed_bytes + block_bytes_ <= max_mb && !should_flush;
    if (is_last && early_last_ && !(next_fits && num_literals < max_literals && num_commands < max_commands)) {
      is_last = false;
      needs_empty_last_ = true;
    }
    if (!is_last && next_fits && num_literals < max_literals && num_commands < max_commands) {
      leave_block();
      if (batch_end) break;
      k = k1 + 1;
      continue;
    }
    MetaBlockPlan mb{};
    if (last_insert_len > 0) {
      trailing_.push_back({k1, last_insert_len});
      num_commands++;
      mb_cmds++;
      num_literals += last_insert_len;
      last_insert_len = 0;
    }
    mb.start = last_flush_pos;
    mb.end = be;
    mb.n_cmds = (uint32_t)mb_cmds;
    mb.n_literals = (uint32_t)num_literals;
    mb.is_last = is_last && stream_is_last_;
    mb.cmd_offset = mb_first_seg;
    memcpy(mb.saved_dist_cache, saved_cache, sizeof(saved_cache));
    const uint32_t bytes = mb.end - mb.start;
    bool compress = true;
    if (num_commands < (uint64_t)(bytes >> 8) + 2 && (float)num_literals > 0.99f * (float)bytes) {
      auto key = std::make_pair(mb.start, bytes);
      auto it = should_compress_cache.find(key);
      if (it == should_compress_cache.end()) {
        wanted_histograms_.push_back(key);
        compress = should_compress_guess_;
        wanted_guesses_.push_back(compress ? 1 : 0);
      } else {
        compress = it->second;
      }
      should_compress_guess_ = compress;
    }
    if (std::find(forced_uncompressed_.begin(), forced_uncompressed_.end(), (uint32_t)metablocks_.size()) !=
        forced_uncompressed_.end())
      compress = false;
    mb.uncompressed = !compress;
    if (!compress) memcpy(cache, saved_cache, sizeof(cache));
    memcpy(mb.dist_cache_after, cache, sizeof(cache));
    mb.dict_lookups_after = dict.L;
    mb.dict_matches_after = dict.M;
    mb.dict_dead_after = dict.state == DictTracker::kDead || dict.state == DictTracker::kUnknown || (dict.use && dict.M < (dict.L >> 7));
    metablocks_.push_back(mb);
    resume_pos_ = be;
    memcpy(saved_cache, cache, sizeof(cache));
    num_commands = 0;
    num_literals = 0;
    mb_cmds = 0;
    last_cmd.valid = false;
    last_flush_pos = be;
    mb_first_seg = k1 + 1;
    k = k1 + 1;
    leave_block();
  }
  block_records_.swap(records);
  block_records_valid_ = true;
  if (block_touched_.size() != nblocks) block_touched_.assign(nblocks, 0);
  dict_death_seg_ = dict.left_alive_at;
  dict_flips_ = dict.flips;
  final_dict_lookups_ = dict.L;
  final_dict_matches_ = dict.M;
  final_dict_dead_ = dict.state == DictTracker::kDead || dict.state == DictTracker::kUnknown;
  return consistent;
}

void Lz77Stage::Warmup(uint32_t first_seg, bool dict_dead, int which, int rbuf, const std::vector<uint8_t>* only_after_dirty) {
  WarmupJob job;
  WarmupBegin(&job, first_seg, (uint32_t)segments_.size(), dict_dead, which, rbuf, only_after_dirty, 3);
  WarmupEnd(&job);
}

void Lz77Stage::WarmupBegin(WarmupJob* job, uint32_t first_seg, uint32_t end_seg, bool dict_dead, int which, int rbuf,
                            const std::vector<uint8_t>* only_after_dirty, int mark) {
  const uint32_t nseg = (uint32_t)segments_.size();
  job->count = 0;
  job->dict_dead = dict_dead;
  job->whole_input = only_after_dirty == nullptr;
  job->mark = mark;
  if (first_seg + 1 >= nseg) return;
  std::vector<uint32_t>& ks = job->ks;
  ks.clear();
  for (uint32_t k = first_seg; k + 1 < nseg && k < end_seg; ++k)
    if (!only_after_dirty || ((*only_after_dirty)[k] && (*only_after_dirty)[k + 1])) ks.push_back(k);
  const uint32_t count = (uint32_t)ks.size();
  job->count = count;
  if (count == 0) return;
  PinnedArray<Segment>& wsegs = job->wsegs;
  PinnedArray<SegEntry>& wentries = job->wentries;
  PinnedArray<SegExit>& wexits = job->wexits;
  wsegs.resize_discard(count);
  wentries.resize_discard(count);
  wexits.resize_discard(count);
  for (uint32_t i = 0; i < count; ++i) {
    const uint32_t k = ks[i];
    Segment g = segments_[k];
    const uint32_t len = g.end - g.start;
    if (len > warmup_bytes_) g.start = g.end - warmup_bytes_;
    g.flags = (g.flags & kSegTailStitched) | kSegWarmup;
    wsegs[i] = g;
    SegEntry e = entries_[k];
    e.pos = g.start;
    e.apply = g.start + P_.spree_window;
    e.dict_lookups = dict_dead ? DictTracker::kDeadL : DictTracker::kAliveL;
    e.dict_matches = dict_dead ? DictTracker::kDeadM : DictTracker::kAliveM;
    wentries[i] = e;
  }
  timeline().stamp("wu-prepared");
  Segment* wsegs_dev = job->mem.zeroed<Segment>(count * sizeof(Segment));
  SegEntry* wentries_dev = job->mem.zeroed<SegEntry>(count * sizeof(SegEntry));
  SegExit* wexits_dev = job->mem.zeroed<SegExit>(count * sizeof(SegExit));
  dev_h2d(wsegs_dev, wsegs.data(), count * sizeof(Segment));
  dev_h2d(wentries_dev, wentries.data(), count * sizeof(SegEntry));
  lz77_parse_custom(P_, B_, which, rbuf, wsegs_dev, wentries_dev, wexits_dev, count);
  timeline().stamp("wu-queued");
  dev_d2h_async(wexits.data(), wexits_dev, count * sizeof(SegExit));
  dev_mark_n(mark);
}

void Lz77Stage::WarmupEnd(WarmupJob* job) {
  const uint32_t nseg = (uint32_t)segments_.size();
  const uint32_t count = job->count;
  if (count == 0) return;
  const std::vector<uint32_t>& ks = job->ks;
  PinnedArray<Segment>& wsegs = job->wsegs;
  PinnedArray<SegEntry>& wentries = job->wentries;
  PinnedArray<SegExit>& wexits = job->wexits;
  const bool dict_dead = job->dict_dead;
  const bool only_after_dirty = !job->whole_input;
  dev_wait_mark_n(job->mark);
  timeline().stamp("wu-exits");
  job->mem.clear();
  if (!dict_dead && !only_after_dirty) {
    if (warm_lookups_.size() != nseg || ks[0] == 0) {
      warm_lookups_.assign(nseg, 0.0);
      warm_matches_.assign(nseg, 0.0);
    }
    for (uint32_t i = 0; i < count; ++i) {
      const double scale = (double)(segments_[ks[i]].end - segments_[ks[i]].start) / (double)(wsegs[i].end - wsegs[i].start);
      warm_lookups_[ks[i]] = scale * (double)(wexits[i].dict_lookups - wentries[i].dict_lookups);
      warm_matches_[ks[i]] = scale * (double)(wexits[i].dict_matches - wentries[i].dict_matches);
    }
  }
  for (uint32_t i = 0; i < count; ++i) {
    SegEntry& e = entries_[ks[i] + 1];
    const uint32_t np = std::min<uint32_t>(wexits[i].n_pushes, 4);
    int32_t guess[4];
    for (uint32_t c = 0; c < 4; ++c) guess[c] = c < np ? wexits[i].cache[c] : entries_[ks[i]].cache[c - np];
    memcpy(e.cache, guess, sizeof(e.cache));
    if (!(segments_[ks[i] + 1].flags & kSegFirstInBlock)) {
      e.pos = wexits[i].pos;
      e.apply = wexits[i].apply;
      e.head_kind = wexits[i].tail_kind;
      e.head_base = wexits[i].tail_base;
      e.head_p1 = wexits[i].tail_p1;
    } else {
      const SegExit& x = wexits[i];
      e.ext_allowed = 0;
      if (x.n_cmds > 0 && x.insert_len == 0 && x.pos >= segments_[ks[i]].blk_end) {
        const uint64_t cmd_dist = (uint64_t)(int64_t)x.cache[0];
        if (x.last_dist_code < 16 || (uint64_t)x.last_dist_code - 15 == cmd_dist) {
          const uint64_t lpp = (uint64_t)segments_[ks[i] + 1].blk_start - x.last_copy_len;
          if (cmd_dist <= std::min<uint64_t>(lpp, P_.max_backward_limit)) e.ext_allowed = 1;
        }
      }
    }
  }
  static const bool no_spree_guess = getenv("BROTLI_MI355X_NO_SPREE_GUESS") != nullptr;
  if (!only_after_dirty && !no_spree_guess) {
    for (uint32_t i = 0; i < count; ++i) {
      const uint32_t k = ks[i];
      if (wexits[i].n_cmds != 0) continue;
      if (segments_[k + 1].flags & kSegFirstInBlock) continue;
      SegEntry from = entries_[k];
      if (segments_[k].flags & kSegFirstInBlock) {
        if (from.ext_allowed) continue;
        from.pos = segments_[k].blk_start;
        from.apply = from.pos + P_.spree_window;
        from.head_kind = kHeadNone;
        from.head_base = from.head_p1 = 0;
      }
      SegExit x{};
      PredictLiteralRun(P_, segments_[k], from, &x);
      SegEntry& e = entries_[k + 1];
      e.pos = x.pos;
      e.apply = x.apply;
      e.head_kind = x.tail_kind;
      e.head_base = x.tail_base;
      e.head_p1 = x.tail_p1;
    }
  }
  stats_.segments_parsed += (uint64_t)count * warmup_bytes_ / segment_bytes_;
  touch_all_ = true;
}

uint32_t Lz77Stage::RecheckCacheOnly(int which, std::vector<uint32_t>* accepted) {
  if (P_.hasher_kind == 9) return 0;
  const uint32_t nseg = (uint32_t)segments_.size();
  std::vector<CacheCheck> items;
  for (uint32_t k = 0; k < nseg; ++k) {
    if (!dirty_entry_[k] || entry_reason_[k] != 2) continue;
    const SegExit& x = exits_[k];
    if (x.n_cmds != 0 || x.ext_len != 0 || x.n_pushes != 0) continue;
    CacheCheck c;
    c.segment = k;
    memcpy(c.cache, next_entries_[k].cache, sizeof(c.cache));
    items.push_back(c);
  }
  if (items.empty()) return 0;
  const uint32_t count = (uint32_t)items.size();
  DevBlocks tmp;
  CacheCheck* items_dev = tmp.zeroed<CacheCheck>(count * sizeof(CacheCheck) + 64);
  uint8_t* ok_dev = tmp.zeroed<uint8_t>(count + 64);
  dev_h2d(items_dev, items.data(), count * sizeof(CacheCheck));
  lz77_check_cache(P_, B_, which, items_dev, count, ok_dev);
  std::vector<uint8_t> ok(count);
  dev_d2h(ok.data(), ok_dev, count);
  tmp.clear();
  uint32_t cleared = 0;
  for (uint32_t i = 0; i < count; ++i) {
    if (!ok[i]) continue;
    const uint32_t k = items[i].segment;
    memcpy(entries_[k].cache, items[i].cache, sizeof(items[i].cache));
    TouchSegment(k);
    if (accepted) accepted->push_back(k);
    dirty_entry_[k] = 0;
    ++cleared;
  }
  return cleared;
}

namespace {
struct Timer {
  bool on;
  std::chrono::steady_clock::time_point t0;
  explicit Timer(bool enabled) : on(enabled) {
    if (on) {
      dev_sync();
      t0 = std::chrono::steady_clock::now();
    }
  }
  void stop(double* acc) {
    if (!on) return;
    dev_sync();
    auto t1 = std::chrono::steady_clock::now();
    *acc += std::chrono::duration<double, std::milli>(t1 - t0).count();
    t0 = t1;
  }
};
}

void Lz77Stage::Run() {
  stats_ = Lz77Stats{};
  const bool prof = getenv("BROTLI_MI355X_PROFILE") != nullptr;
  Timer total(true);
  Timer tm(prof);
  should_compress_cache_.clear();
  block_records_valid_ = false;
  touch_all_ = true;
  resolve_incremental_ = false;
  const uint32_t nseg = (uint32_t)segments_.size();
  if (nseg == 0) {
    metablocks_.clear();
    total_cmds_ = 0;
    return;
  }
  if (use_zopfli_ || use_quick_) {
    if (use_quick_) { if (use_qspec_) RunQuickSpec(); else RunQuick(); } else RunZopfli();
    tm.stop(&stats_.ms_parse);
    Gather();
    tm.stop(&stats_.ms_gather);
    total.stop(&stats_.ms_total);
    return;
  }
  lz77_compute_keys(P_, B_);
  tm.stop(&stats_.ms_keys);
  lz77_sort_by_key(P_, B_);
  key_first_.resize_discard(65537);
  key_last_.resize_discard(65537);
  dev_d2h_async(key_first_.data(), B_.key_first, 65537 * 4);
  dev_d2h_async(key_last_.data(), B_.key_last, 65537 * 4);
  uint32_t run_samples = 0;
  dev_d2h_async(&run_samples, B_.changed_count + 8, 4);
  timeline().stamp("sort-queued");
  dev_sync();
  timeline().stamp("sorted");
  if (run_samples >= 64 && getenv("BROTLI_MI355X_NO_RUN_TABLE") == nullptr) {
    if (!B_.run_end) B_.run_end = mem_.uninit<uint32_t>((size_t)P_.total_bytes * 4 + 64);
    lz77_run_table(P_, B_);
    if (getenv("BROTLI_MI355X_SELFTEST")) {
      const uint32_t n = P_.total_bytes;
      std::vector<uint32_t> got(n);
      std::vector<uint8_t> text(n);
      dev_d2h(got.data(), B_.run_end, (size_t)n * 4);
// ... 496 lines not shown
    lz77_scatter_entries(B_, list_dev, up_entries_dev, count);
    if (own) lz77_qspec_block_tables(P_, B_, Q_, S_, list_dev, count, own_tables, own_stride);
    lz77_qspec_parse(P_, B_, Q_, S_, list_dev, count, own ? own_tables : nullptr, own_stride);
    lz77_qspec_gather_exits(B_, list_dev, count, got_exits_dev);
    if (own) {
      lz77_qspec_first_change(B_, S_, list_dev, count, first_change_dev);
      dev_d2h_async(first_change.data(), first_change_dev, 4);
    }
    diffed = !never_incremental && !own;
    if (diffed) {
      lz77_qspec_diff(P_, B_, Q_, S_, list_dev, count);
      dev_d2h_async(chg_count.data(), S_.chg_count, 64);
    }
    dev_d2h(R.got_exits.data(), got_exits_dev, (size_t)count * sizeof(SegExit));
    for (uint32_t i = 0; i < count; ++i) exits_[R.up_index[i]] = R.got_exits[i];
  }
  stats_.incremental_ranks += incremental_rounds;
  stamp("qs-settled");
  if (settled && selftest) {
    const size_t words = (size_t)S_.n * Q_.sweep;
    std::vector<uint32_t> kept(words), fresh(words);
    dev_d2h(kept.data(), S_.cand, words * 4);
    lz77_qspec_candidates(P_, B_, Q_, S_, nullptr, nullptr);
    dev_d2h(fresh.data(), S_.cand, words * 4);
    for (size_t i = 0; i < words; ++i)
      if (kept[i] != fresh[i])
        throw std::runtime_error("selftest: candidate " + std::to_string(i % Q_.sweep) + " of position " + std::to_string(i / Q_.sweep) + " is " + std::to_string(kept[i]) +
                                 " after the repairs of " + std::to_string(incremental_rounds) + " rounds, " + std::to_string(fresh[i]) + " from the final flags");
  }
  tmp.clear();
  if (restart_coarse) {
    saved_block_guess_.clear();
    for (uint32_t k = 0; k < nseg; ++k)
      if (segments_[k].flags & kSegFirstInBlock) saved_block_guess_[segments_[k].blk_start] = next_entries_[k];
    if (debug) fprintf(stderr, "quick: the parse does not fall into step inside the blocks, one chain per block from here\n");
    coarse_blocks_.assign(block_segment_bytes_.size(), 1);
    Resegment(segment_bytes_);
    qspec_coarse_ = true;
    stats_.coarse_restarts++;
    RunQuickSpec();
    return;
  }
  if (!settled) {
    if (debug) fprintf(stderr, "quick: not settled after %u rounds, the serial path takes over\n", (unsigned)dirty_history.size());
    use_qspec_ = false;
    P_.use_dictionary = 0;
    Resegment(block_bytes_);
    mem_.drop(B_.entries);
    mem_.drop(B_.exits);
    mem_.drop(gather_offsets_dev_);
    mem_.drop(gather_counts_dev_);
    B_.entries = mem_.zeroed<SegEntry>(segments_.size() * sizeof(SegEntry) + 64);
    B_.exits = mem_.zeroed<SegExit>(segments_.size() * sizeof(SegExit) + 64);
    gather_offsets_dev_ = mem_.zeroed<uint32_t>(segments_.size() * 4 + 64);
    gather_counts_dev_ = mem_.zeroed<uint32_t>(segments_.size() * 4 + 64);
    stats_.coarse_restarts++;
    RunQuick();
    return;
  }
  final_flags_ = 0;
  for (uint32_t k = 0; k < nseg; ++k) stats_.searches += exits_[k].n_searches;
}

void Lz77Stage::RunZopfli() {
  const bool debug = getenv("BROTLI_MI355X_DEBUG") != nullptr;
  const uint32_t nseg = (uint32_t)segments_.size();
  if (P_.reset_pos != 0) throw std::runtime_error("brotli_mi355x: quality 10 / 11 across the reference's 32-bit position wrap is not supported");
  InitEntries();
  lz77_compute_keys(P_, B_);
  lz77_sort_by_key(P_, B_);
  const size_t forest_bytes = ((size_t)2 << Z_.lgwin) * 4, bucket_bytes = ((size_t)1 << 17) * 4;
  if (carry_ && carry_->valid && carry_->zopfli) {
    const ZopfliCarry& zc = *carry_->zopfli;
    if (zc.lgwin != Z_.lgwin || carry_->stream_base < zc.text_base) throw std::runtime_error("brotli_mi355x: quality 10 / 11: the carried trees do not fit this piece");
    lz77_zopfli_import(Z_, zc.buckets, zc.forest, (uint32_t)(carry_->stream_base - zc.text_base));
  } else {
    lz77_zopfli_init(Z_);
    if (P_.prefix_bytes > 1) lz77_zopfli_prepend(P_, B_, Z_, P_.prefix_bytes);
  }
  bool starts_metablock = true;
  uint32_t from = 0;
  bool done = false;
  for (uint32_t round = 0; round < nseg + 8 && !done; ++round) {
    stats_.rounds++;
    if (round != 0) entries_[from] = next_entries_[from];
    if (partial_ && starts_metablock) {
      if (!zsnap_buckets_) {
        zsnap_buckets_ = mem_.uninit<uint32_t>(bucket_bytes + 64);
        zsnap_forest_ = mem_.uninit<uint32_t>(forest_bytes + 64);
      }
      dev_d2d(zsnap_buckets_, Z_.buckets, bucket_bytes);
      dev_d2d(zsnap_forest_, Z_.forest, forest_bytes);
    }
    dev_h2d(B_.entries + from, entries_.data() + from, sizeof(SegEntry));
    if (lz77_zopfli_block(P_, B_, Z_, from)) stats_.coarse_restarts++;
    stats_.segments_parsed++;
    dev_d2h(exits_.data() + from, B_.exits + from, sizeof(SegExit));
    if (exits_[from].bad_commands != 0)
      throw std::runtime_error("brotli_mi355x: the reference encoder fails on this input at quality 10 / 11 (it indexes past the end of an array)");
    Resolve(false);
    for (uint32_t k = 0; k <= from; ++k)
      if (dirty_entry_[k]) throw std::runtime_error("brotli_mi355x: resolver and Zopfli parse disagree about the entry of a finished block");
    if (debug) fprintf(stderr, "zopfli block %u of %u done: %u commands, %u bytes pending\n", from, nseg, exits_[from].n_cmds, exits_[from].insert_len);
    starts_metablock = false;
    for (const MetaBlockPlan& mb : metablocks_)
      if (mb.end == segments_[from].blk_end) starts_metablock = true;
    ++from;
    done = from == nseg;
  }
  if (!done) throw std::runtime_error("brotli_mi355x: quality 10 / 11 parse did not finish");
  if (partial_ && starts_metablock) {
    if (!zsnap_buckets_) {
      zsnap_buckets_ = mem_.uninit<uint32_t>(bucket_bytes + 64);
      zsnap_forest_ = mem_.uninit<uint32_t>(forest_bytes + 64);
    }
    dev_d2d(zsnap_buckets_, Z_.buckets, bucket_bytes);
    dev_d2d(zsnap_forest_, Z_.forest, forest_bytes);
  }
  final_flags_ = 0;
  for (uint32_t k = 0; k < nseg; ++k) stats_.searches += exits_[k].n_searches;
}

void Lz77Stage::RunRounds(bool allow_restart) {
  if (use_live_) {
    RunLive();
    return;
  }
  const bool prof = getenv("BROTLI_MI355X_PROFILE") != nullptr;
  Timer tm(prof);
  const uint32_t nseg = (uint32_t)segments_.size();
  resolve_incremental_ = true;
  block_records_valid_ = false;
  touch_all_ = true;
  block_touched_.assign(block_segment_bytes_.size(), 0);
  InitFlags();
  tm.stop(&stats_.ms_init);
  const bool selftest = getenv("BROTLI_MI355X_SELFTEST") != nullptr;
  const bool selftest_rows_every_update = getenv("BROTLI_MI355X_SELFTEST_ROWS") != nullptr;
  if (selftest) SelfTestSort();
  int which = 0, rbuf = 0;
  {
    RankInitialHint hint{segments_[0].blk_start, block_bytes_, (carry_ && carry_->valid) ? 0u : 1u};
    if (use_rows_) {
      lz77_rows_init(P_, B_, which, &hint, has_big_keys_);
    } else {
      lz77_rank_flags(P_, B_, which, rbuf, &hint);
    }
  }
  InitEntries();
  tm.stop(&stats_.ms_rank);
  timeline().stamp("index-queued");
  if (selftest) {
    if (use_rows_) SelfTestRows(which); else SelfTestRank(which, rbuf);
  }
  if (const char* w = getenv("BROTLI_MI355X_WARMUP")) warmup_bytes_ = (uint32_t)atoi(w);
  double fc_L = 0, fc_M = 0;
  uint32_t fc_death = nseg;
  bool fc_found = false;
  auto forecast = [&](uint32_t from, uint32_t upto) {
    if (!(P_.use_dictionary && warm_lookups_.size() == nseg)) return;
    const double sample = (double)warmup_bytes_ / (double)segment_bytes_;
    for (uint32_t k = from; k < upto && !fc_found; ++k) {
      fc_L += warm_lookups_[k];
      fc_M += warm_matches_[k];
      const double sigma = std::sqrt(std::max(1.0, fc_M * sample)) / sample;
      if (fc_L >= 256.0 && fc_M + 3.0 * sigma < fc_L / 128.0) {
        fc_death = k;
        fc_found = true;
      }
    }
    if (upto == nseg || fc_found) {
      for (uint32_t k = fc_death + 1; k < nseg; ++k) {
        entries_[k].dict_lookups = DictTracker::kDeadL;
        entries_[k].dict_matches = DictTracker::kDeadM;
      }
      touch_all_ = true;
      predicted_death_ = fc_death;
    }
  };
  if (nseg > 1 && warmup_bytes_ > 0) {
    Warmup(0, false, which, rbuf, nullptr);
    timeline().stamp("warmed-up");
    forecast(0, nseg);
    tm.stop(&stats_.ms_warmup);
  }
  if (!allow_restart && !saved_block_guess_.empty()) {
    for (uint32_t k = 0; k < nseg; ++k) {
      if (!(segments_[k].flags & kSegFirstInBlock)) continue;
      auto it = saved_block_guess_.find(segments_[k].blk_start);
      if (it == saved_block_guess_.end()) continue;
      memcpy(entries_[k].cache, it->second.cache, sizeof(entries_[k].cache));
      entries_[k].ext_allowed = it->second.ext_allowed;
      touch_all_ = true;
    }
  }
  SegGeometry geo{};
  geo.prefix_bytes = P_.prefix_bytes;
  geo.first_block_start = segments_[0].blk_start;
  geo.block_bytes = block_bytes_;
  geo.num_blocks = (uint32_t)block_segment_bytes_.size();
  DevBlocks tmp;
  uint32_t* geo_tables = tmp.zeroed<uint32_t>((block_first_segment_.size() + block_segment_bytes_.size()) * 4 + 64);
  dev_h2d(geo_tables, block_first_segment_.data(), block_first_segment_.size() * 4);
  dev_h2d(geo_tables + block_first_segment_.size(), block_segment_bytes_.data(), block_segment_bytes_.size() * 4);
  geo.block_first_segment = geo_tables;
  geo.block_segment_bytes = geo_tables + block_first_segment_.size();
  geo.num_segments = nseg;
  geo.block_size = 1u << P_.block_bits;
  uint8_t* dirty_dev = tmp.zeroed<uint8_t>(nseg + 64);
  uint32_t* list_dev = tmp.zeroed<uint32_t>((size_t)nseg * 8 + 64);
  std::vector<uint8_t> dirty(nseg, 0);
  std::vector<uint32_t> list(nseg);
  static constexpr uint32_t kContFirst = 64;
  const uint32_t cont_cap = std::max(nseg, kContFirst);
  SegEntry* up_entries_dev = tmp.uninit<SegEntry>((size_t)nseg * 2 * sizeof(SegEntry) + 64);
  SegExit* got_exits_dev = tmp.uninit<SegExit>((size_t)nseg * sizeof(SegExit) + 64);
  uint32_t* cont_count_dev = tmp.zeroed<uint32_t>(64);
  uint32_t* cont_index_dev = tmp.zeroed<uint32_t>((size_t)cont_cap * 4 + 64);
  SegExit* cont_exits_dev = tmp.uninit<SegExit>((size_t)cont_cap * sizeof(SegExit) + 64);
  SegEntry* cont_entries_dev = tmp.uninit<SegEntry>((size_t)cont_cap * sizeof(SegEntry) + 64);
  std::vector<uint32_t> also_upload;
  static const uint32_t burst_env = getenv("BROTLI_MI355X_BURST") ? (uint32_t)atoi(getenv("BROTLI_MI355X_BURST")) : 8u;
  static const uint32_t splice_max_share = getenv("BROTLI_MI355X_SPLICE_SHARE") ? (uint32_t)atoi(getenv("BROTLI_MI355X_SPLICE_SHARE")) : 8u;
  static const uint32_t burst_shrink = getenv("BROTLI_MI355X_BURST_SHRINK") ? (uint32_t)atoi(getenv("BROTLI_MI355X_BURST_SHRINK")) : 4u;
  const uint32_t burst_max = (use_rows_ && B_.run_end == nullptr) ? burst_env : 0u;
  BurstBuffers U;
  bool stale_marks_valid = false;
  if (burst_max != 0) {
    U.sched = tmp.zeroed<uint8_t>(nseg + 64);
    U.cand_dirty = dirty_dev;
    U.entry_dirty = tmp.zeroed<uint8_t>(nseg + 64);
    U.touched = tmp.zeroed<uint8_t>(nseg + 64);
    U.stale = tmp.zeroed<uint8_t>(nseg + 64);
    U.new_entries = tmp.uninit<SegEntry>((size_t)nseg * sizeof(SegEntry) + 64);
    U.list = tmp.uninit<uint32_t>((size_t)nseg * 4 + 64);
    U.counters = tmp.zeroed<uint32_t>(64);
  }
  RoundBuffers& rb = round_buffers_;
  rb.up_index.resize_discard((size_t)nseg * 2);
  rb.up_entries.resize_discard((size_t)nseg * 2);
  rb.got_exits.resize_discard(nseg);
  rb.cont_index.resize_discard(cont_cap);
  rb.cont_exits.resize_discard(cont_cap);
  rb.cont_entries.resize_discard(cont_cap);
  rb.counts.resize_discard(4);
  uint32_t* up_index = rb.up_index.data();
  SegEntry* up_entries = rb.up_entries.data();
  SegExit* got_exits = rb.got_exits.data();
  uint32_t* cont_index = rb.cont_index.data();
  SegExit* cont_exits = rb.cont_exits.data();
  SegEntry* cont_entries = rb.cont_entries.data();
  volatile uint32_t* counts = rb.counts.data();
  const bool debug = getenv("BROTLI_MI355X_DEBUG") != nullptr;
  std::vector<uint32_t> changed_all(kChangedCap);
  std::vector<uint8_t> entry_streak(nseg, 0), was_dirty, cand_dirty, pending(nseg, 0), sched(nseg, 0);
  std::vector<uint8_t> cache_wave(nseg, 0), cache_wave_next(nseg, 0);
  const bool follow_cache_fronts = getenv("BROTLI_MI355X_NO_CACHE_FRONTS") == nullptr;
  for (uint32_t k = 0; k < nseg; ++k) list[k] = k;
  uint32_t count = nseg;
  const uint32_t max_rounds = getenv("BROTLI_MI355X_MAX_ROUNDS") ? (uint32_t)atoi(getenv("BROTLI_MI355X_MAX_ROUNDS")) : nseg + 8;
  bool done = false;
  bool restart = false;
  bool full_round = true;
  uint32_t last_death_seg = 0xffffffffu;
  auto stamp = [&](const char* what) { timeline().stamp(what); };
  for (uint32_t round = 0; round < max_rounds && !done; ++round) {
    stats_.rounds++;
    stamp("| round");
    tm.stop(&stats_.ms_resolve);
    if (full_round) {
      dev_h2d(B_.entries, entries_.data(), (size_t)nseg * sizeof(SegEntry));
    } else {
      const uint32_t n_up = count + (uint32_t)also_upload.size();
      for (uint32_t i = 0; i < n_up; ++i) {
        up_index[i] = i < count ? list[i] : also_upload[i - count];
        up_entries[i] = entries_[up_index[i]];
      }
      dev_h2d(list_dev, up_index, (size_t)n_up * 4);
      dev_h2d(up_entries_dev, up_entries, (size_t)n_up * sizeof(SegEntry));
      lz77_scatter_entries(B_, list_dev, up_entries_dev, n_up);
      if (n_up > count) lz77_drop_checkpoints(P_, B_, list_dev + count, n_up - count);
      dev_h2d(burst_max != 0 ? U.sched : dirty_dev, sched.data(), nseg);
    }
    also_upload.clear();
    const bool burst = !full_round && burst_max != 0;
    uint32_t n_touched = 0;
    if (burst) {
      const uint32_t* launch_list = list_dev;
      uint32_t launch_count = count;
      for (uint32_t it = 0;; ++it) {
        B_.splice_lists = (uint64_t)launch_count * splice_max_share <= nseg ? 1u : 0u;
        if (stale_marks_valid) {
          lz77_flags_catch_up(P_, B_, U, which, which ^ 1);
        } else {
          dev_d2d(B_.flags[which ^ 1], B_.flags[which], (size_t)P_.total_bytes + 64);
          dev_memset(U.stale, 0, nseg);
          stale_marks_valid = true;
        }
        lz77_parse_list(P_, B_, which, rbuf, launch_list, U.sched, launch_count);
        stats_.segments_parsed += launch_count;
        lz77_chain_check(P_, B_, U);
        lz77_diff_flags_touched(P_, B_, U, which, which ^ 1);
        dev_memset(dirty_dev, 0, nseg);
        lz77_rows_update(P_, B_, which, which ^ 1, geo, dirty_dev, has_big_keys_);
        which ^= 1;
        stats_.burst_launches++;
        if (selftest_rows_every_update) SelfTestRows(which);
        if (it + 1 >= burst_max) break;
        lz77_burst_count(P_, B_, U);
        dev_d2h((void*)counts, U.counters, 4);
        const uint32_t next_count = counts[0];
        if (debug) fprintf(stderr, "  burst launch %u: %u segments next\n", it, next_count);
        if (next_count == 0 || (uint64_t)next_count * burst_shrink > launch_count) break;
        lz77_burst_schedule(P_, B_, U);
        launch_list = U.list;
        launch_count = next_count;
      }
      which ^= 1;
      lz77_gather_touched(P_, B_, U, cont_index_dev, cont_exits_dev, cont_entries_dev);
      dev_d2h((void*)counts, U.counters, 8);
      n_touched = counts[1];
      dev_d2h_async(cont_index, cont_index_dev, (size_t)n_touched * 4);
      dev_d2h_async(cont_exits, cont_exits_dev, (size_t)n_touched * sizeof(SegExit));
      dev_d2h_async(cont_entries, cont_entries_dev, (size_t)n_touched * sizeof(SegEntry));
      dev_sync();
      stamp("burst-done");
    } else {
    dev_d2d(B_.flags[which ^ 1], B_.flags[which], (size_t)P_.total_bytes + 64);
    stamp("uploaded");
    if (full_round) {
      lz77_parse_round(P_, B_, which, rbuf, 0);
    } else {
      lz77_parse_list(P_, B_, which, rbuf, list_dev, dirty_dev, count);
    }
    stats_.segments_parsed += count;
    lz77_diff_flags(P_, B_, which, which ^ 1);
    }
    if (getenv("BROTLI_MI355X_DEBUG_FLAGS")) {
      std::vector<uint8_t> fa(P_.total_bytes), fb(P_.total_bytes);
      dev_d2h(fa.data(), B_.flags[which], P_.total_bytes);
      dev_d2h(fb.data(), B_.flags[which ^ 1], P_.total_bytes);
      uint32_t shown = 0;
      for (uint32_t q = 0; q < P_.total_bytes && shown < 40; ++q)
        if ((fa[q] ^ fb[q]) & 1) {
          fprintf(stderr, "  flag change at %u (seg %u, off %u): %u -> %u\n", q, q / segment_bytes_, q % segment_bytes_, fa[q], fb[q]);
          shown++;
        }
    }
    if (burst) {
      for (uint32_t i = 0; i < n_touched; ++i) {
        const uint32_t k = cont_index[i];
        pending[k] = 0;
        exits_[k] = cont_exits[i];
        entries_[k] = cont_entries[i];
        TouchSegment(k);
      }
      counts[0] = 1;
      counts[1] = 0;
    } else {
    counts[0] = counts[1] = 0;
    if (full_round) {
      dev_d2h_async(exits_.data(), B_.exits, (size_t)nseg * sizeof(SegExit));
      touch_all_ = true;
    } else {
      lz77_gather_results(B_, list_dev, count, dirty_dev, nseg, got_exits_dev, cont_count_dev, cont_index_dev, cont_exits_dev, cont_entries_dev);
      dev_d2h_async(got_exits, got_exits_dev, (size_t)count * sizeof(SegExit));
      dev_d2h_async((void*)(counts + 1), cont_count_dev, 4);
      dev_d2h_async(cont_index, cont_index_dev, (size_t)kContFirst * 4);
      dev_d2h_async(cont_exits, cont_exits_dev, (size_t)kContFirst * sizeof(SegExit));
      dev_d2h_async(cont_entries, cont_entries_dev, (size_t)kContFirst * sizeof(SegEntry));
    }
    dev_d2h_async((void*)counts, B_.changed_count, 4);
    if (!use_rows_) dev_d2h_async(changed_all.data(), B_.changed_keys, (size_t)kChangedCap * 4);
    if (use_rows_) {
      dev_mark();
      dev_memset(dirty_dev, 0, nseg);
      stamp("launched");
      if (full_round) lz77_reset_rows_changed(P_, B_);
      lz77_rows_update(P_, B_, which, which ^ 1, geo, dirty_dev, has_big_keys_);
      stamp("rows-queued");
      dev_wait_mark();
      stamp("exits-here");
    } else {
      dev_sync();
    }
    }
    const uint32_t n_changed = counts[0], n_cont = counts[1];
    if (!full_round && !burst) {
      for (uint32_t i = 0; i < count; ++i) {
        exits_[list[i]] = got_exits[i];
        TouchSegment(list[i]);
      }
      if (n_cont > kContFirst) {
        dev_d2h(cont_index, cont_index_dev, (size_t)n_cont * 4);
        dev_d2h(cont_exits, cont_exits_dev, (size_t)n_cont * sizeof(SegExit));
        dev_d2h(cont_entries, cont_entries_dev, (size_t)n_cont * sizeof(SegEntry));
      }
      if (debug) fprintf(stderr, "  continued into %u segments\n", n_cont);
      for (uint32_t i = 0; i < n_cont; ++i) {
        const uint32_t k = cont_index[i];
        pending[k] = 0;
        exits_[k] = cont_exits[i];
        entries_[k] = cont_entries[i];
        TouchSegment(k);
        cache_wave[k] = 1;
        stats_.segments_parsed++;
      }
    }
    tm.stop(&stats_.ms_parse);
    which ^= 1;
    if (selftest_rows_every_update && use_rows_) SelfTestRows(which);
    if (use_rows_) {
      if (n_changed != 0) (n_changed <= B_.changed_cap ? stats_.incremental_ranks : stats_.full_ranks)++;
    } else if (n_changed != 0) {
      std::vector<uint32_t> changed;
      bool incremental = false;
      if (n_changed <= kChangedCap) {
        changed.assign(changed_all.begin(), changed_all.begin() + n_changed);
        std::sort(changed.begin(), changed.end());
        changed.erase(std::unique(changed.begin(), changed.end()), changed.end());
        uint64_t affected = 0;
        uint32_t widest = 0;
        for (uint32_t key : changed) {
          const uint32_t width = key_last_[key] - key_first_[key];
          affected += width;
          widest = std::max(widest, width);
        }
        (void)widest;
        static const uint32_t inc_pct = getenv("BROTLI_MI355X_INC_PCT") ? (uint32_t)atoi(getenv("BROTLI_MI355X_INC_PCT")) : 100u;
        incremental = affected <= (uint64_t)P_.total_bytes * inc_pct / 100;
      }
      dev_memset(dirty_dev, 0, nseg);
      if (B_.recheck_count) dev_memset(B_.recheck_count, 0, 4);
      if (incremental) {
        std::vector<RerankChunk> chunks;
        for (uint32_t key : changed) {
          const uint32_t lo = key_first_[key], hi = key_last_[key];
          const uint32_t first_sum = (uint32_t)chunks.size();
          for (uint32_t b = lo; b < hi; b += kRerankChunk)
            chunks.push_back({lo, b, std::min(hi, b + kRerankChunk), first_sum, (uint32_t)chunks.size()});
        }
        RerankChunk* chunks_dev = tmp.zeroed<RerankChunk>(chunks.size() * sizeof(RerankChunk) + 64);
        uint32_t* sums_dev = tmp.zeroed<uint32_t>(chunks.size() * 4 + 64);
        dev_h2d(chunks_dev, chunks.data(), chunks.size() * sizeof(RerankChunk));
        lz77_rerank_keys(P_, B_, which, rbuf, chunks_dev, (uint32_t)chunks.size(), sums_dev, geo, dirty_dev);
        tmp.drop(chunks_dev);
        tmp.drop(sums_dev);
        stats_.incremental_ranks++;
      } else {
        lz77_rank_flags(P_, B_, which, rbuf ^ 1);
        lz77_validate(P_, B_, which, rbuf, rbuf ^ 1, geo, dirty_dev);
        rbuf ^= 1;
        stats_.full_ranks++;
      }
      lz77_recheck_searches(P_, B_, rbuf, geo, dirty_dev);
    }
    tm.stop(&stats_.ms_rank);
    if (const char* path = getenv("BROTLI_MI355X_DEBUG_FRONT")) {
      if (FILE* f = fopen(path, "a")) {
        uint32_t front = 0;
        while (!was_dirty.empty() && front < nseg && !was_dirty[front]) ++front;
        fprintf(f, "R %u %u", round, front);
        for (uint32_t k = front; k < nseg && k < front + 24; ++k)
          fprintf(f, " %u:%u:%u:%u", k, exits_[k].pos, exits_[k].n_cmds, round == 0 ? 1u : (uint32_t)sched[k]);
        fprintf(f, "\n");
        fclose(f);
      }
    }
    const auto host_t0 = std::chrono::steady_clock::now();
    Resolve(false);
    const auto host_t1 = std::chrono::steady_clock::now();
    host_resolve_ms_ += std::chrono::duration<double, std::milli>(host_t1 - host_t0).count();
    stamp("resolved");
    const uint32_t rechecked = RecheckCacheOnly(which, &also_upload);
    stamp("rechecked");
    stats_.cache_rechecks += rechecked;
    for (uint32_t k = 0; k < nseg; ++k) dirty[k] = dirty_entry_[k] | pending[k];
    uint32_t n_dirty_entry = 0, n_dirty_valid = 0;
    for (uint32_t k = 0; k < nseg; ++k) n_dirty_entry += dirty[k];
    if (round == 0 && allow_restart && segment_bytes_ < block_bytes_ && nseg >= 64 && (uint64_t)(dbg_counts_[0] - std::min(dbg_counts_[0], predicted_runs_)) * 2 > nseg) {
      coarse_blocks_.assign(block_segment_bytes_.size(), 1);
      restart = true;
      break;
    }
    cand_dirty.clear();
    if (n_changed != 0) {
      cand_dirty.resize(nseg);
      dev_d2h(cand_dirty.data(), dirty_dev, nseg);
      for (uint32_t k = 0; k < nseg; ++k) {
        n_dirty_valid += cand_dirty[k];
        dirty[k] |= cand_dirty[k];
      }
      tm.stop(&stats_.ms_rank);
      stamp("dirty-here");
    }
    const bool regime_flip = dict_death_seg_ != 0xffffffffu && dict_death_seg_ != last_death_seg && dict_flips_ > 64;
    for (uint32_t k = 0; k < nseg; ++k) entry_streak[k] = dirty_entry_[k] ? (uint8_t)std::min<uint32_t>(entry_streak[k] + 1u, 255u) : (uint8_t)0;
    if (const char* first = getenv("BROTLI_MI355X_DEBUG_MAP")) {
      const uint32_t a = std::max<uint32_t>((uint32_t)atoi(first), 0u) ? (uint32_t)atoi(first) : 16u;
      std::string m;
      for (uint32_t k = a; k < a + 32 && k < nseg; ++k) m += dirty_entry_[k] ? (pending[k] ? 'P' : 'E') : (dirty[k] ? 'c' : '.');
      fprintf(stderr, "  map[%u..%u) %s\n", a, a + 32, m.c_str());
      for (uint32_t k = a; k < a + 12 && k < nseg; ++k)
        fprintf(stderr, "    seg %u [%u,%u) used pos %u apply %u head %u/%u cache %d %d %d %d | chained pos %u apply %u head %u/%u cache %d %d %d %d | exit pos %u cmds %u searches %u\n",
                k, segments_[k].start, segments_[k].end, entries_[k].pos, entries_[k].apply, entries_[k].head_kind, entries_[k].head_base,
                entries_[k].cache[0], entries_[k].cache[1], entries_[k].cache[2], entries_[k].cache[3], next_entries_[k].pos,
                next_entries_[k].apply, next_entries_[k].head_kind, next_entries_[k].head_base, next_entries_[k].cache[0],
                next_entries_[k].cache[1], next_entries_[k].cache[2], next_entries_[k].cache[3], exits_[k].pos, exits_[k].n_cmds,
                exits_[k].n_searches);
    }
    if (const char* path = getenv("BROTLI_MI355X_DEBUG_DIRTY")) {
      if (FILE* f = fopen(path, "a")) {
        std::string m(nseg, '.');
        for (uint32_t k = 0; k < nseg; ++k) {
          const bool c = !cand_dirty.empty() && cand_dirty[k];
          m[k] = dirty_entry_[k] ? (c ? 'B' : (pending[k] ? 'P' : 'E')) : (c ? 'c' : (dirty[k] ? 'p' : '.'));
        }
        std::string why(nseg, '0');
        for (uint32_t k = 0; k < nseg; ++k) why[k] = (char)('0' + (entry_reason_[k] & 3));
        fprintf(f, "%s %s\n", m.c_str(), why.c_str());
        fclose(f);
      }
    }
    was_dirty = dirty;
    const bool aggressive = false;
    count = 0;
    bool front_run = false;
    cache_wave_next.assign(nseg, 0);
    for (uint32_t k = 0; k < nseg; ++k) {
      sched[k] = 0;
      if (segments_[k].flags & kSegFirstInBlock) front_run = false;
      if (!dirty[k]) {
        front_run = false;
        continue;
      }
      const bool must_redo = pending[k] || (!cand_dirty.empty() && cand_dirty[k]);
      if (front_run && !dirty_entry_[k]) {
        sched[k] = 2;
        pending[k] = 1;
        dirty[k] = 0;
// ... 305 lines not shown
```

rust-brotli_amd/csrc/lz77_stage.h:

```cpp
#ifndef BROTLI_MI355X_LZ77_STAGE_H_
#define BROTLI_MI355X_LZ77_STAGE_H_

#include <stdint.h>
#include <map>
#include <memory>
#include <utility>
#include <vector>

#include "device_api.h"
#include "encoder_params.h"
#include "quick_api.h"

namespace brotli_mi355x {

struct MetaBlockPlan {
  uint32_t start;
  uint32_t end;
  uint32_t cmd_offset;
  uint32_t n_cmds;
  uint32_t n_literals;
  bool uncompressed;
  bool is_last;
  int32_t dist_cache_after[4];
  int32_t saved_dist_cache[4];
  uint32_t dict_lookups_after, dict_matches_after;
  bool dict_dead_after;
};

struct Lz77Stats {
  uint32_t rounds = 0;
  uint64_t segments_parsed = 0;
  uint64_t searches = 0;
  uint64_t total_commands = 0;
  uint32_t incremental_ranks = 0, full_ranks = 0, coarse_restarts = 0;
  uint32_t burst_launches = 0;
  uint64_t cache_rechecks = 0;
  double ms_keys = 0, ms_sort = 0, ms_init = 0, ms_warmup = 0, ms_rank = 0, ms_parse = 0, ms_resolve = 0, ms_gather = 0, ms_total = 0;
};

struct ZopfliCarry {
  DevBlocks mem;
  uint32_t* buckets = nullptr;
  uint32_t* forest = nullptr;
  uint32_t lgwin = 0;
  uint64_t text_base = 0;
};

struct QuickCarry {
  DevBlocks mem;
  uint32_t* table = nullptr;
  uint64_t text_base = 0;
};

struct StreamCarry {
  bool valid = false;
  int32_t dist_cache[4] = {4, 11, 15, 16};
  uint32_t dict_lookups = 0, dict_matches = 0;
  bool dict_dead = false;
  std::vector<uint8_t> stored;
  HasherParams hasher;
  size_t size_hint = 0;
  uint64_t stream_base = 0;
  std::vector<uint32_t> key_counts;
  uint32_t tail_bits = 0, tail_nbits = 0;
  uint32_t dict_break = 0;
  bool use_dictionary = true;
  uint32_t prev_floor = 0;
  uint32_t catable_raw_bytes = 0;
  std::shared_ptr<ZopfliCarry> zopfli;
  std::shared_ptr<QuickCarry> quick;
  bool magic_owed = false;
};

class Lz77Stage {
 public:
  Lz77Stage() = default;
  Lz77Stage(const Lz77Stage&) = delete;
  Lz77Stage& operator=(const Lz77Stage&) = delete;

  void Setup(const EncoderParams& params, uint8_t* text_dev, uint32_t prefix_bytes, uint32_t input_bytes,
             uint32_t raw_head_bytes, uint32_t segment_bytes);
  void ForceUncompressed(uint32_t index) { forced_uncompressed_.push_back(index); }
  void SetStreamState(const StreamCarry* carry, bool stream_is_last, bool partial = false, bool last_block_processed_early = false) {
    carry_ = carry;
    stream_is_last_ = stream_is_last;
    partial_ = partial;
    early_last_ = last_block_processed_early && stream_is_last;
  }
  bool needs_empty_last() const { return needs_empty_last_; }
  uint32_t resume_pos() const { return resume_pos_; }
  void SetHasherReset(uint32_t pos) {
    P_.reset_pos = pos;
    P_.reset_vis = pos >= 3 ? pos - 3 : 0;
  }
  void KeyCountsBetween(uint32_t from, uint32_t upto, std::vector<uint32_t>* out);
  void KeyCountsBefore(uint32_t upto, std::vector<uint32_t>* out);
  void ExportZopfli(StreamCarry* co, bool partial);
  bool is_zopfli() const { return use_zopfli_; }
  void ExportQuick(StreamCarry* co, bool partial);
  bool is_quick() const { return use_quick_; }
  void FinalDictState(uint32_t* lookups, uint32_t* matches, bool* dead) const {
    *lookups = final_dict_lookups_;
    *matches = final_dict_matches_;
    *dead = final_dict_dead_;
  }
  uint32_t total_bytes() const { return P_.total_bytes; }
  void set_warmup_bytes(uint32_t n) { warmup_bytes_ = n; }
  void Run();
  void DumpFlags(uint8_t* out, size_t size) const;

  const std::vector<MetaBlockPlan>& metablocks() const { return metablocks_; }
  Command* commands_dev() const { return gathered_cmds_; }
  uint32_t num_commands() const { return (uint32_t)total_cmds_; }
  const Lz77Stats& stats() const { return stats_; }
  const Lz77Params& device_params() const { return P_; }
  const uint8_t* text_dev() const { return B_.text; }

 private:
  void BuildSegments();
  void Resegment(uint32_t segment_bytes);
  void RunRounds(bool allow_restart);
  void RunLive();
  void RunZopfli();
  void RunQuick();
  void RunQuickSpec();
  void InitEntries();
  void InitFlags();
  bool Resolve(bool final_pass);
  void Gather();
  struct WarmupJob {
    std::vector<uint32_t> ks;
    PinnedArray<Segment> wsegs;
    PinnedArray<SegEntry> wentries;
    PinnedArray<SegExit> wexits;
    DevBlocks mem;
    uint32_t count = 0;
    bool dict_dead = false, whole_input = true;
    int mark = 0;
  };
  void Warmup(uint32_t first_seg, bool dict_dead, int which, int rbuf, const std::vector<uint8_t>* only_after_dirty);
  void WarmupBegin(WarmupJob* job, uint32_t first_seg, uint32_t end_seg, bool dict_dead, int which, int rbuf,
                   const std::vector<uint8_t>* only_after_dirty, int mark);
  void WarmupEnd(WarmupJob* job);
  void SelfTestSort();
  void SelfTestRank(int which, int rbuf);
  void SelfTestRows(int which);
  bool FetchShouldCompress();
  bool ResolvePass(bool final_pass, bool incremental);
  void SetupCommon(bool with_sort_tmp);
  void Release();

  EncoderParams params_;
  Lz77Params P_{};
  DevBlocks mem_;
  Lz77Buffers B_{};
  LiveBuffers L_{};
  bool use_live_ = false;
  bool use_zopfli_ = false;
  ZopfliJob Z_{};
  uint32_t* zsnap_buckets_ = nullptr;
  uint32_t* zsnap_forest_ = nullptr;
  bool use_quick_ = false;
  QuickJob Q_{};
  uint32_t* qsnap_table_ = nullptr;
  bool use_qspec_ = false;
  QuickSpec S_{};
  EncoderParams qspec_params_{};
  uint8_t* qspec_text_ = nullptr;
  uint32_t qspec_prefix_ = 0, qspec_input_ = 0, qspec_raw_head_ = 0;
  bool qspec_coarse_ = false;
  bool qspec_books_in_ = false;
  uint32_t qspec_lookups_ = 0, qspec_matches_ = 0;
  bool live_verify_ = false;
  std::vector<LiveBlockState> live_state_;
  uint32_t input_bytes_ = 0;
  uint32_t raw_head_bytes_ = 0;
  uint32_t segment_bytes_ = 4096;
  uint32_t warmup_bytes_ = 384;
  uint32_t block_bytes_ = 65536;
  std::vector<Segment> segments_;
  std::vector<uint32_t> block_first_segment_, block_segment_bytes_;
  std::vector<uint8_t> coarse_blocks_;
  uint32_t total_cmd_slots_ = 0;
  std::vector<double> warm_lookups_, warm_matches_;
  uint32_t predicted_death_ = 0xffffffffu;
  int final_flags_ = 0;
  const StreamCarry* carry_ = nullptr;
  bool stream_is_last_ = true;
  bool partial_ = false;
  bool early_last_ = false, needs_empty_last_ = false;
  uint32_t resume_pos_ = 0;
  uint32_t final_dict_lookups_ = 0, final_dict_matches_ = 0;
  bool final_dict_dead_ = false;
  std::map<uint32_t, SegEntry> saved_block_guess_;
  size_t cmds_bytes_ = 0;
  PinnedArray<uint32_t> key_first_, key_last_;
  PinnedArray<Segment> segments_upload_;
  PinnedArray<SegEntry> entries_;
  std::vector<SegEntry> next_entries_;
  PinnedArray<SegExit> exits_;
  struct RoundBuffers {
    PinnedArray<uint32_t> up_index, cont_index, counts;
    PinnedArray<SegEntry> up_entries, cont_entries;
    PinnedArray<SegExit> got_exits, cont_exits;
  } round_buffers_;
  std::vector<MetaBlockPlan> metablocks_;
  std::vector<uint32_t> forced_uncompressed_;
  struct Patch {
    uint32_t segment;
    uint32_t index;
    uint32_t ext;
  };
  std::vector<Patch> patches_;
  struct TrailingInsert {
    uint32_t after_segment;
    uint32_t insert_len;
  };
  std::vector<TrailingInsert> trailing_;
  struct Carry {
    uint32_t segment;
    uint32_t literals;
  };
  std::vector<Carry> carries_;
  Command* gathered_cmds_ = nullptr;
  size_t gathered_capacity_ = 0;
  size_t total_cmds_ = 0;
  uint32_t* histo_dev_ = nullptr;
  uint32_t* gather_offsets_dev_ = nullptr;
  uint32_t* gather_counts_dev_ = nullptr;
  Lz77Stats stats_;
  uint32_t dbg_counts_[4] = {0, 0, 0, 0};
  uint32_t dbg_first_[4] = {0, 0, 0, 0};
  uint32_t* dbg_mismatch_ = nullptr;
  std::map<std::pair<uint32_t, uint32_t>, bool> should_compress_cache_;
  std::vector<uint8_t> wanted_guesses_;
  bool should_compress_guess_ = true;
  std::vector<std::pair<uint32_t, uint32_t>> wanted_histograms_;
  uint32_t first_dirty_ = 0;
  std::vector<uint8_t> predicted_entry_;
  std::vector<uint8_t> entry_reason_;
  bool substitute_inherited_pushes_ = false;
  uint32_t RecheckCacheOnly(int which, std::vector<uint32_t>* accepted = nullptr);
  double host_resolve_ms_ = 0, host_schedule_ms_ = 0;
  uint32_t predicted_runs_ = 0;
  struct ResolveFlow {
    int32_t cache[4], saved_cache[4];
    uint32_t last_insert_len, last_flush_pos, mb_first_seg, resume_pos;
    uint64_t num_commands, num_literals, mb_cmds;
    uint32_t dict_state, dict_L, dict_M, dict_left_alive_at, dict_flips;
    int64_t dict_slack;
    uint32_t last_valid, last_seg, last_idx, last_dist_code, last_copy_len;
    uint32_t compress_guess, needs_empty_last;
  };
  struct ResolveBlockRecord {
    ResolveFlow in;
    uint32_t n_metablocks, n_patches, n_trailing, n_carries;
    uint32_t marks, first_dirty, predicted_runs;
    uint32_t dbg_counts[4], dbg_first[4];
    uint32_t merged_ext;
  };
  std::vector<ResolveBlockRecord> block_records_;
  std::vector<MetaBlockPlan> metablocks_prev_;
  std::vector<Patch> patches_prev_;
  std::vector<TrailingInsert> trailing_prev_;
  std::vector<Carry> carries_prev_;
  std::vector<uint8_t> block_touched_;
  bool block_records_valid_ = false, touch_all_ = true, resolve_incremental_ = false;
  uint32_t resolve_blocks_skipped_ = 0;
  void TouchSegment(uint32_t k) {
    if (!block_touched_.empty()) block_touched_[segments_[k].block_index] = 1;
  }
  std::vector<uint8_t> dirty_entry_;
  uint32_t dict_death_seg_ = 0xffffffffu;
  uint32_t dict_flips_ = 0;
  uint32_t* count_base_dev_ = nullptr;
  bool use_rows_ = false;
  bool has_big_keys_ = false;
};

}
#endif
```

Before: 4465 MB/s.

## Move warmup entry composition to device scans and widen the key-hashing kernel

Segment warmup entries (distance cache composition, dictionary death detection, literal-spree propagation) are now computed on the GPU. A tiled associative scan over per-segment warmup ops replaces the host-side sequential loop and its host/device transfers. Separately, k_compute_keys is rewritten to process four bytes per thread with 1024-thread workgroups, with packed word loads, an LDS copy of the dictionary hash table, vectorised stores and a double-buffered histogram. The changes add several kernel launches, alignment requirements, and a serial spree walk inside k_warmup_finish that could become long for some inputs.

```diff
diff --git a/rust-brotli_amd/csrc/device_api.h b/rust-brotli_amd/csrc/device_api.h
--- a/rust-brotli_amd/csrc/device_api.h
+++ b/rust-brotli_amd/csrc/device_api.h
@@ -7,6 +7,7 @@
 #include <vector>
 
 #include "lz77_types.h"
+#include "lz77_warmup.h"
 
 #define BR_STREAM (::brotli_mi355x::dev_stream_flushed())
 
@@ -201,6 +202,15 @@
 void lz77_parse_round(const Lz77Params& P, const Lz77Buffers& B, int which, int rbuf, uint32_t first_segment);
 void lz77_parse_list(const Lz77Params& P, const Lz77Buffers& B, int which, int rbuf, const uint32_t* list_dev, uint8_t* sched_dev,
                      uint32_t count);
+struct WarmupBuffers {
+  Segment* segs;
+  SegEntry* entries;
+  SegExit* exits;
+  WarmupOp* tile_ops;
+  uint32_t* fc_death;
+};
+void lz77_warmup_prepare(const Lz77Params& P, const Lz77Buffers& B, const WarmupShape& S, const WarmupBuffers& W, const int32_t base_cache[4]);
+void lz77_warmup_compose(const Lz77Params& P, const Lz77Buffers& B, const WarmupShape& S, const WarmupBuffers& W);
 void lz77_scatter_entries(const Lz77Buffers& B, const uint32_t* index_dev, const SegEntry* entries_dev, uint32_t count);
 void lz77_gather_results(const Lz77Buffers& B, const uint32_t* list_dev, uint32_t count, const uint8_t* sched_dev, uint32_t num_segments,
                          SegExit* exits_out, uint32_t* cont_count, uint32_t* cont_index, SegExit* cont_exits, SegEntry* cont_entries);
diff --git a/rust-brotli_amd/csrc/lz77_kernels.hip b/rust-brotli_amd/csrc/lz77_kernels.hip
--- a/rust-brotli_amd/csrc/lz77_kernels.hip
+++ b/rust-brotli_amd/csrc/lz77_kernels.hip
@@ -25,53 +25,80 @@
 
 static constexpr uint32_t kSortTile = 4096;
 
-__global__ __launch_bounds__(256) void k_compute_keys(const uint8_t* __restrict__ text, uint16_t* __restrict__ keys,
-                                                      uint32_t n, uint32_t valid_n, uint32_t kind, uint32_t bucket_bits,
-                                                      uint64_t hash_mask, uint32_t* __restrict__ run_samples,
-                                                      const uint16_t* __restrict__ dict_hash, uint32_t* __restrict__ dict_items,
-                                                      uint32_t num_tiles, uint32_t* __restrict__ hist) {
-  __shared__ uint32_t h[256];
-  for (uint32_t tile = blockIdx.x; tile < num_tiles; tile += gridDim.x) {
-    const uint32_t tile_base = tile * kSortTile;
-    const uint32_t tile_n = n - tile_base < kSortTile ? n - tile_base : kSortTile;
-    if (hist != nullptr) {
-      h[threadIdx.x] = 0;
-      __syncthreads();
-    }
-#pragma unroll 4
-    for (uint32_t e = threadIdx.x; e < tile_n; e += 256) {
-      const uint32_t i = tile_base + e;
-      if (dict_items != nullptr) {
-        const uint32_t dh = ((br_load32(text + i) * 0x1e35a7bdu) >> (32 - 14)) << 1;
-        dict_items[i] = (uint32_t)dict_hash[dh] | ((uint32_t)dict_hash[dh + 1] << 16);
+static constexpr uint32_t kKeysThreads = 1024;
+static_assert(kKeysThreads * 4 == kSortTile, "one sort tile per step of a workgroup");
+
+__global__ __launch_bounds__(kKeysThreads) void k_compute_keys(const uint8_t* __restrict__ text, uint16_t* __restrict__ keys,
+                                                               uint32_t n, uint32_t valid_n, uint32_t kind, uint32_t bucket_bits,
+                                                               uint64_t hash_mask, uint32_t* __restrict__ run_samples,
+                                                               const uint16_t* __restrict__ dict_hash, uint32_t* __restrict__ dict_items,
+                                                               uint32_t num_tiles, uint32_t* __restrict__ hist) {
+  __shared__ uint32_t tab[16384];
+  __shared__ uint32_t h[2][256];
+  const uint32_t t = threadIdx.x;
+  if (dict_items != nullptr) {
+    const uint4* src = (const uint4*)dict_hash;
+    for (uint32_t q = t; q < 4096; q += kKeysThreads) ((uint4*)tab)[q] = src[q];
+  }
+  if (t < 512) (&h[0][0])[t] = 0;
+  __syncthreads();
+  const uint32_t mis = (uint32_t)((uintptr_t)text & 3u), sh = 8 * mis;
+  const uint32_t* text32 = (const uint32_t*)(text - mis);
+  uint32_t b = 0;
+  for (uint32_t tile = blockIdx.x; tile < num_tiles; tile += gridDim.x, b ^= 1u) {
+    const uint32_t i = tile * kSortTile + 4 * t;
+    if (i < n) {
+      uint32_t w0 = text32[i >> 2], w1 = text32[(i >> 2) + 1], w2 = text32[(i >> 2) + 2];
+      if (mis != 0) {
+        const uint32_t w3 = text32[(i >> 2) + 3];
+        w0 = (w0 >> sh) | (w1 << (32 - sh));
+        w1 = (w1 >> sh) | (w2 << (32 - sh));
+        w2 = (w2 >> sh) | (w3 << (32 - sh));
       }
-      uint32_t key = 0xffffu;
-      if (i < valid_n) {
-        if ((i & 63u) == 0 && i + 16 <= n) {
-          const uint64_t v = br_load64(text + i);
-          if (v == (v & 0xffull) * 0x0101010101010101ull && br_load64(text + i + 8) == v && *(volatile uint32_t*)run_samples < 4096u)
-            atomicAdd(run_samples, 1u);
+      if ((i & 63u) == 0 && i < valid_n && i + 16 <= n) {
+        if (w0 == (w0 & 0xffu) * 0x01010101u && w1 == w0 && w2 == w0 && br_load32(text + i + 12) == w0 && *(volatile uint32_t*)run_samples < 4096u)
+          atomicAdd(run_samples, 1u);
+      }
+      uint32_t key[4], item[4];
+#pragma unroll
+      for (uint32_t j = 0; j < 4; ++j) {
+        const uint32_t lo = j ? (w0 >> (8 * j)) | (w1 << (32 - 8 * j)) : w0;
+        const uint32_t hi = j ? (w1 >> (8 * j)) | (w2 << (32 - 8 * j)) : w1;
+        item[j] = dict_items != nullptr ? tab[(lo * 0x1e35a7bdu) >> (32 - 14)] : 0u;
+        uint32_t k = 0xffffu;
+        if (i + j < valid_n) {
+          if (kind == 6) {
+            const uint64_t v = ((((uint64_t)hi << 32) | lo) & hash_mask) * 0x1fe35a7bd3579bd3ull;
+            k = (uint32_t)(v >> (64 - bucket_bits)) & 0xffffu;
+          } else {
+            k = ((lo * 0x1e35a7bdu) >> (32 - bucket_bits)) & 0xffffu;
+          }
         }
-        if (kind == 6) {
-          const uint64_t v = (br_load64(text + i) & hash_mask) * 0x1fe35a7bd3579bd3ull;
-          key = (uint32_t)(v >> (64 - bucket_bits));
-        } else {
-          const uint32_t v = br_load32(text + i) * 0x1e35a7bdu;
-          key = v >> (32 - bucket_bits);
+        key[j] = k;
+        if (hist != nullptr && i + j < n) atomicAdd(&h[b][k & 255u], 1u);
+      }
+      if (i + 4 <= n) {
+        *(uint2*)(keys + i) = make_uint2(key[0] | (key[1] << 16), key[2] | (key[3] << 16));
+        if (dict_items != nullptr) *(uint4*)(dict_items + i) = make_uint4(item[0], item[1], item[2], item[3]);
+      } else {
+#pragma unroll
+        for (uint32_t j = 0; j < 4; ++j) {
+          if (i + j >= n) break;
+          keys[i + j] = (uint16_t)key[j];
+          if (dict_items != nullptr) dict_items[i + j] = item[j];
         }
       }
-      keys[i] = (uint16_t)key;
-      if (hist != nullptr) atomicAdd(&h[key & 255u], 1u);
     }
     if (hist != nullptr) {
       __syncthreads();
-      hist[threadIdx.x * num_tiles + tile] = h[threadIdx.x];
-    }
-  }
-  if (dict_items != nullptr && blockIdx.x == 0 && threadIdx.x == 0) {
-    const uint32_t dh = ((br_load32(text + n) * 0x1e35a7bdu) >> (32 - 14)) << 1;
-    dict_items[n] = (uint32_t)dict_hash[dh] | ((uint32_t)dict_hash[dh + 1] << 16);
-  }
+      if (t < 256) {
+        hist[t * num_tiles + tile] = h[b][t];
+        h[b][t] = 0;
+      }
+    }
+  }
+  if (dict_items != nullptr && blockIdx.x == 0 && t == 0)
+    dict_items[n] = tab[(br_load32(text + n) * 0x1e35a7bdu) >> (32 - 14)];
 }
 
 struct SortScratch {
@@ -104,8 +131,16 @@
   if (n == 0) return;
   const uint32_t tiles = (n + kSortTile - 1) / kSortTile;
   uint32_t* hist = (B.sort_tmp != nullptr && B.sort_tmp_bytes >= lz77_sort_tmp_bytes(n)) ? sort_scratch(B, n).hist : nullptr;
+  if (((uintptr_t)B.keys & 7) || ((uintptr_t)B.dict_items & 15))
+    throw std::runtime_error("brotli_mi355x: lz77_compute_keys needs keys aligned to 8 and dict_items to 16 bytes");
+  static const uint32_t workgroups = [] {
+    int dev = 0, cus = 0;
+    HIP_CHECK(hipGetDevice(&dev));
+    HIP_CHECK(hipDeviceGetAttribute(&cus, hipDeviceAttributeMultiprocessorCount, dev));
+    return cus > 0 ? 2u * (uint32_t)cus : 512u;
+  }();
   dev_memset(B.changed_count + 8, 0, 4);
-  hipLaunchKernelGGL(k_compute_keys, dim3(tiles < 8192 ? tiles : 8192), dim3(256), 0, BR_STREAM, B.text, B.keys, n, valid_n, P.hasher_kind,
+  hipLaunchKernelGGL(k_compute_keys, dim3(tiles < workgroups ? tiles : workgroups), dim3(kKeysThreads), 0, BR_STREAM, B.text, B.keys, n, valid_n, P.hasher_kind,
                      P.bucket_bits, hash_mask, B.changed_count + 8, dev_tables().dict_hash, B.dict_items, tiles, hist);
   HIP_CHECK(hipGetLastError());
 }
@@ -1565,6 +1600,150 @@
   launch_parse(P, B, which, which ^ 1, rbuf, segments_dev, entries_dev, exits_dev, 0, nullptr, nullptr, count);
 }
 
+__global__ __launch_bounds__(kWarmupTile) void k_warmup_prepare(const Segment* __restrict__ segments, SegEntry* __restrict__ entries,
+                                                                uint32_t num_segments, uint32_t warmup_bytes, uint32_t spree_window,
+                                                                int32_t c0, int32_t c1, int32_t c2, int32_t c3, WarmupBuffers W) {
+  const uint32_t k = blockIdx.x * kWarmupTile + threadIdx.x;
+  if (k >= num_segments) return;
+  if (k == 0) W.fc_death[0] = num_segments;
+  const Segment g = segments[k];
+  SegEntry e{};
+  e.pos = g.start;
+  e.apply = g.start + spree_window;
+  e.cache[0] = c0;
+  e.cache[1] = c1;
+  e.cache[2] = c2;
+  e.cache[3] = c3;
+  if (k != 0) {
+    e.dict_lookups = kWarmAliveL;
+    e.dict_matches = kWarmAliveM;
+  }
+  entries[k] = e;
+  if (k + 1 < num_segments) {
+    const Segment dry = warmup_segment(g, warmup_bytes);
+    W.segs[k] = dry;
+    W.entries[k] = warmup_entry(e, dry, spree_window, false);
+  }
+}
+
+__device__ __forceinline__ WarmupOp warmup_block_scan(WarmupOp v, WarmupOp* sh) {
+  const uint32_t t = threadIdx.x;
+  uint32_t cur = 0;
+  __syncthreads();
+  sh[t] = v;
+  __syncthreads();
+  for (uint32_t off = 1; off < kWarmupTile; off <<= 1) {
+    WarmupOp r = sh[cur * kWarmupTile + t];
+    if (t >= off) r = warmup_combine(sh[cur * kWarmupTile + t - off], r);
+    cur ^= 1u;
+    sh[cur * kWarmupTile + t] = r;
+    __syncthreads();
+  }
+  return sh[cur * kWarmupTile + t];
+}
+
+__device__ __forceinline__ WarmupOp warmup_op_of(const Segment* segments, const WarmupBuffers& W, uint32_t i, uint32_t count, uint32_t warmup_bytes) {
+  if (i >= count) return warmup_identity();
+  return warmup_op(segments[i], W.exits[i], W.entries[i].dict_lookups, W.entries[i].dict_matches, warmup_bytes);
+}
+
+__global__ __launch_bounds__(kWarmupTile) void k_warmup_tile_ops(const Segment* __restrict__ segments, WarmupShape S, WarmupBuffers W) {
+  __shared__ WarmupOp sh[2 * kWarmupTile];
+  const uint32_t count = S.num_segments - 1;
+  const WarmupOp o = warmup_block_scan(warmup_op_of(segments, W, blockIdx.x * kWarmupTile + threadIdx.x, count, S.warmup_bytes), sh);
+  if (threadIdx.x == kWarmupTile - 1) W.tile_ops[blockIdx.x] = o;
+}
+
+__global__ __launch_bounds__(kWarmupTile) void k_warmup_tile_carry(uint32_t tiles, WarmupBuffers W) {
+  __shared__ WarmupOp sh[2 * kWarmupTile];
+  __shared__ WarmupOp carry;
+  if (threadIdx.x == 0) carry = warmup_identity();
+  for (uint32_t base = 0; base < tiles; base += kWarmupTile) {
+    const uint32_t i = base + threadIdx.x;
+    const WarmupOp own = i < tiles ? W.tile_ops[i] : warmup_identity();
+    const WarmupOp incl = warmup_block_scan(own, sh);
+    const WarmupOp upto = warmup_combine(carry, incl);
+    __syncthreads();
+    sh[threadIdx.x] = upto;
+    __syncthreads();
+    if (i < tiles) W.tile_ops[tiles + i] = threadIdx.x == 0 ? carry : sh[threadIdx.x - 1];
+    __syncthreads();
+    if (threadIdx.x == kWarmupTile - 1) carry = upto;
+  }
+}
+
+__global__ __launch_bounds__(kWarmupTile) void k_warmup_entries(const Segment* __restrict__ segments, SegEntry* __restrict__ entries,
+                                                                WarmupShape S, uint32_t max_backward_limit, uint32_t use_dictionary,
+                                                                uint32_t tiles, WarmupBuffers W) {
+  __shared__ WarmupOp sh[2 * kWarmupTile];
+  const uint32_t count = S.num_segments - 1;
+  const uint32_t i = blockIdx.x * kWarmupTile + threadIdx.x;
+  const WarmupOp incl = warmup_block_scan(warmup_op_of(segments, W, i, count, S.warmup_bytes), sh);
+  if (i >= count) return;
+  const WarmupOp upto = warmup_combine(W.tile_ops[tiles + blockIdx.x], incl);
+  SegEntry e = entries[i + 1];
+  int32_t base[4];
+  for (int c = 0; c < 4; ++c) base[c] = entries[0].cache[c];
+  warmup_apply_cache(upto, base, e.cache);
+  warmup_entry_from_exit(segments[i], segments[i + 1], W.exits[i], max_backward_limit, &e);
+  entries[i + 1] = e;
+  if (use_dictionary && warmup_dictionary_dies(upto.sl, upto.sm, S.warmup_bytes, S.segment_bytes)) atomicMin(W.fc_death, i);
+}
+
+__global__ __launch_bounds__(kWarmupTile) void k_warmup_finish(const Segment* __restrict__ segments, SegEntry* __restrict__ entries,
+                                                               WarmupShape S, uint32_t htl, uint32_t spree_window, uint32_t use_dictionary,
+                                                               WarmupBuffers W) {
+  const uint32_t k = blockIdx.x * kWarmupTile + threadIdx.x;
+  if (k >= S.num_segments) return;
+  if (use_dictionary && k > W.fc_death[0]) {
+    entries[k].dict_lookups = kWarmDeadL;
+    entries[k].dict_matches = kWarmDeadM;
+  }
+  const uint32_t count = S.num_segments - 1;
+  if (!S.spree_guess || k >= count) return;
+  auto carries = [&](uint32_t j) {
+    SegEntry probe{};
+    probe.ext_allowed = entries[j].ext_allowed;
+    return warmup_spree_carries(segments[j], segments[j + 1], probe, W.exits[j]);
+  };
+  if (!carries(k) || (k > 0 && carries(k - 1))) return;
+  SegEntry cur{};
+  cur.pos = entries[k].pos;
+  cur.apply = entries[k].apply;
+  cur.head_kind = entries[k].head_kind;
+  cur.head_base = entries[k].head_base;
+  cur.head_p1 = entries[k].head_p1;
+  for (uint32_t j = k; j < count && (j == k || carries(j)); ++j) {
+    SegEntry next{};
+    warmup_spree_step(htl, spree_window, segments[j], cur, &next);
+    entries[j + 1].pos = next.pos;
+    entries[j + 1].apply = next.apply;
+    entries[j + 1].head_kind = next.head_kind;
+    entries[j + 1].head_base = next.head_base;
+    entries[j + 1].head_p1 = next.head_p1;
+    cur = next;
+  }
+}
+
+void lz77_warmup_prepare(const Lz77Params& P, const Lz77Buffers& B, const WarmupShape& S, const WarmupBuffers& W, const int32_t base_cache[4]) {
+  if (S.num_segments == 0) return;
+  hipLaunchKernelGGL(k_warmup_prepare, dim3((S.num_segments + kWarmupTile - 1) / kWarmupTile), dim3(kWarmupTile), 0, BR_STREAM, B.segments,
+                     B.entries, S.num_segments, S.warmup_bytes, P.spree_window, base_cache[0], base_cache[1], base_cache[2], base_cache[3], W);
+  HIP_CHECK(hipGetLastError());
+}
+
+void lz77_warmup_compose(const Lz77Params& P, const Lz77Buffers& B, const WarmupShape& S, const WarmupBuffers& W) {
+  if (S.num_segments < 2) return;
+  const uint32_t tiles = (S.num_segments - 1 + kWarmupTile - 1) / kWarmupTile;
+  hipLaunchKernelGGL(k_warmup_tile_ops, dim3(tiles), dim3(kWarmupTile), 0, BR_STREAM, B.segments, S, W);
+  hipLaunchKernelGGL(k_warmup_tile_carry, dim3(1), dim3(kWarmupTile), 0, BR_STREAM, tiles, W);
+  hipLaunchKernelGGL(k_warmup_entries, dim3(tiles), dim3(kWarmupTile), 0, BR_STREAM, B.segments, B.entries, S, P.max_backward_limit,
+                     P.use_dictionary, tiles, W);
+  hipLaunchKernelGGL(k_warmup_finish, dim3((S.num_segments + kWarmupTile - 1) / kWarmupTile), dim3(kWarmupTile), 0, BR_STREAM, B.segments,
+                     B.entries, S, P.htl, P.spree_window, P.use_dictionary, W);
+  HIP_CHECK(hipGetLastError());
+}
+
 struct FlipCells {
   uint32_t* bits;
   uint32_t shift, per_key, words;
diff --git a/rust-brotli_amd/csrc/lz77_stage.cpp b/rust-brotli_amd/csrc/lz77_stage.cpp
--- a/rust-brotli_amd/csrc/lz77_stage.cpp
+++ b/rust-brotli_amd/csrc/lz77_stage.cpp
@@ -15,6 +15,10 @@
 #include "host_entropy.h"
 
 #include <cmath>
+
+#if defined(BROTLI_HOST_EMU)
+#include "lz77_warmup_emu.inc"
+#endif
 
 namespace brotli_mi355x {
 
@@ -352,8 +356,8 @@
   int64_t slack = 0;
   uint32_t left_alive_at = 0xffffffffu;
   uint32_t flips = 0;
-  static constexpr uint32_t kDeadL = 0x40000000u, kDeadM = 0;
-  static constexpr uint32_t kAliveL = 0, kAliveM = 0x01000000u;
+  static constexpr uint32_t kDeadL = kWarmDeadL, kDeadM = kWarmDeadM;
+  static constexpr uint32_t kAliveL = kWarmAliveL, kAliveM = kWarmAliveM;
   static constexpr int64_t kSlackPerChain = 256;
   void Hint(SegEntry* e) const {
     switch (state) {
@@ -478,39 +482,7 @@
 }
 
 static void PredictLiteralRun(const Lz77Params& P, const Segment& seg, const SegEntry& e, SegExit* x) {
-  const uint64_t pos_end = seg.blk_end, htl = P.htl, window = P.spree_window;
-  const uint64_t margin = htl - 1 > 4 ? htl - 1 : 4;
-  uint64_t position = e.pos;
-  const uint64_t apply = e.apply;
-  uint32_t tail_kind = e.head_kind;
-  uint64_t tail_base = e.head_base;
-  const uint64_t stop = std::min<uint64_t>(pos_end > htl ? pos_end - htl : 0, seg.end);
-  if (position < stop && position < apply) position = std::min(stop, apply);
-  const uint64_t block_tail = pos_end > margin + 16 ? pos_end - margin - 16 : 0;
-  auto stride = [&](uint64_t step, uint64_t p_limit, uint32_t kind) {
-    uint64_t bound = stop;
-    bound = std::min(bound, block_tail > 0 ? block_tail - 1 : 0);
-    bound = std::min(bound, p_limit);
-    if (position >= bound) return;
-    const uint64_t n = (bound - position + step - 1) / step;
-    tail_kind = kind;
-    tail_base = position + (n - 1) * step + 1;
-    position += n * step;
-  };
-  if (position < stop) stride(9, apply + 4 * window, kHeadEven4);
-  if (position < stop && position + 1 > apply + 4 * window) stride(17, ~0ull >> 1, kHeadVec4);
-  if (position < stop && position + 1 >= block_tail && position + 1 > apply) {
-    tail_kind = kHeadUnstored;
-    tail_base = position + 1;
-    position = pos_end;
-  }
-  if (seg.flags & kSegLastInBlock) position = pos_end;
-  x->pos = (uint32_t)position;
-  x->apply = (uint32_t)apply;
-  x->insert_len = (uint32_t)position - e.pos;
-  x->tail_kind = position > seg.end ? tail_kind : (uint32_t)kHeadNone;
-  x->tail_base = position > seg.end ? (uint32_t)tail_base : 0u;
-  x->tail_p1 = position > seg.end ? e.head_p1 : 0u;
+  warmup_predict_literal_run(P.htl, P.spree_window, seg, e, x);
   static const bool selftest = getenv("BROTLI_MI355X_SELFTEST") != nullptr || getenv("BROTLI_MI355X_SELFTEST_RESOLVE") != nullptr;
   if (selftest) {
     SegExit y = *x;
@@ -1007,41 +979,39 @@
   WarmupEnd(&job);
 }
 
-void Lz77Stage::WarmupBegin(WarmupJob* job, uint32_t first_seg, uint32_t end_seg, bool dict_dead, int which, int rbuf,
-                            const std::vector<uint8_t>* only_after_dirty, int mark) {
+uint32_t Lz77Stage::WarmupPlan(WarmupJob* job, uint32_t first_seg, uint32_t end_seg, bool dict_dead, const std::vector<uint8_t>* only_after_dirty) {
   const uint32_t nseg = (uint32_t)segments_.size();
   job->count = 0;
   job->dict_dead = dict_dead;
   job->whole_input = only_after_dirty == nullptr;
-  job->mark = mark;
-  if (first_seg + 1 >= nseg) return;
+  if (first_seg + 1 >= nseg) return 0;
   std::vector<uint32_t>& ks = job->ks;
   ks.clear();
   for (uint32_t k = first_seg; k + 1 < nseg && k < end_seg; ++k)
     if (!only_after_dirty || ((*only_after_dirty)[k] && (*only_after_dirty)[k + 1])) ks.push_back(k);
   const uint32_t count = (uint32_t)ks.size();
   job->count = count;
+  if (count == 0) return 0;
+  job->wsegs.resize_discard(count);
+  job->wentries.resize_discard(count);
+  job->wexits.resize_discard(count);
+  for (uint32_t i = 0; i < count; ++i) {
+    const uint32_t k = ks[i];
+    job->wsegs[i] = warmup_segment(segments_[k], warmup_bytes_);
+    job->wentries[i] = warmup_entry(entries_[k], job->wsegs[i], P_.spree_window, dict_dead);
+  }
+  return count;
+}
+
+void Lz77Stage::WarmupBegin(WarmupJob* job, uint32_t first_seg, uint32_t end_seg, bool dict_dead, int which, int rbuf,
+                            const std::vector<uint8_t>* only_after_dirty, int mark) {
+  job->mark = mark;
+  job->launched = true;
+  const uint32_t count = WarmupPlan(job, first_seg, end_seg, dict_dead, only_after_dirty);
   if (count == 0) return;
   PinnedArray<Segment>& wsegs = job->wsegs;
   PinnedArray<SegEntry>& wentries = job->wentries;
   PinnedArray<SegExit>& wexits = job->wexits;
-  wsegs.resize_discard(count);
-  wentries.resize_discard(count);
-  wexits.resize_discard(count);
-  for (uint32_t i = 0; i < count; ++i) {
-    const uint32_t k = ks[i];
-    Segment g = segments_[k];
-    const uint32_t len = g.end - g.start;
-    if (len > warmup_bytes_) g.start = g.end - warmup_bytes_;
-    g.flags = (g.flags & kSegTailStitched) | kSegWarmup;
-    wsegs[i] = g;
-    SegEntry e = entries_[k];
-    e.pos = g.start;
-    e.apply = g.start + P_.spree_window;
-    e.dict_lookups = dict_dead ? DictTracker::kDeadL : DictTracker::kAliveL;
-    e.dict_matches = dict_dead ? DictTracker::kDeadM : DictTracker::kAliveM;
-    wentries[i] = e;
-  }
   timeline().stamp("wu-prepared");
   Segment* wsegs_dev = job->mem.zeroed<Segment>(count * sizeof(Segment));
   SegEntry* wentries_dev = job->mem.zeroed<SegEntry>(count * sizeof(SegEntry));
@@ -1059,23 +1029,24 @@
   const uint32_t count = job->count;
   if (count == 0) return;
   const std::vector<uint32_t>& ks = job->ks;
-  PinnedArray<Segment>& wsegs = job->wsegs;
   PinnedArray<SegEntry>& wentries = job->wentries;
   PinnedArray<SegExit>& wexits = job->wexits;
   const bool dict_dead = job->dict_dead;
   const bool only_after_dirty = !job->whole_input;
-  dev_wait_mark_n(job->mark);
-  timeline().stamp("wu-exits");
-  job->mem.clear();
+  if (job->launched) {
+    dev_wait_mark_n(job->mark);
+    timeline().stamp("wu-exits");
+    job->mem.clear();
+  }
   if (!dict_dead && !only_after_dirty) {
     if (warm_lookups_.size() != nseg || ks[0] == 0) {
-      warm_lookups_.assign(nseg, 0.0);
-      warm_matches_.assign(nseg, 0.0);
+      warm_lookups_.assign(nseg, 0);
+      warm_matches_.assign(nseg, 0);
     }
     for (uint32_t i = 0; i < count; ++i) {
-      const double scale = (double)(segments_[ks[i]].end - segments_[ks[i]].start) / (double)(wsegs[i].end - wsegs[i].start);
-      warm_lookups_[ks[i]] = scale * (double)(wexits[i].dict_lookups - wentries[i].dict_lookups);
-      warm_matches_[ks[i]] = scale * (double)(wexits[i].dict_matches - wentries[i].dict_matches);
+      const WarmupOp o = warmup_op(segments_[ks[i]], wexits[i], wentries[i].dict_lookups, wentries[i].dict_matches, warmup_bytes_);
+      warm_lookups_[ks[i]] = o.sl;
+      warm_matches_[ks[i]] = o.sm;
     }
   }
   for (uint32_t i = 0; i < count; ++i) {
@@ -1878,47 +1849,6 @@
   timeline().stamp("index-queued");
   if (selftest) {
     if (use_rows_) SelfTestRows(which); else SelfTestRank(which, rbuf);
-  }
-  if (const char* w = getenv("BROTLI_MI355X_WARMUP")) warmup_bytes_ = (uint32_t)atoi(w);
-  double fc_L = 0, fc_M = 0;
-  uint32_t fc_death = nseg;
-  bool fc_found = false;
-  auto forecast = [&](uint32_t from, uint32_t upto) {
-    if (!(P_.use_dictionary && warm_lookups_.size() == nseg)) return;
-    const double sample = (double)warmup_bytes_ / (double)segment_bytes_;
-    for (uint32_t k = from; k < upto && !fc_found; ++k) {
-      fc_L += warm_lookups_[k];
-      fc_M += warm_matches_[k];
-      const double sigma = std::sqrt(std::max(1.0, fc_M * sample)) / sample;
-      if (fc_L >= 256.0 && fc_M + 3.0 * sigma < fc_L / 128.0) {
-        fc_death = k;
-        fc_found = true;
-      }
-    }
-    if (upto == nseg || fc_found) {
-      for (uint32_t k = fc_death + 1; k < nseg; ++k) {
-        entries_[k].dict_lookups = DictTracker::kDeadL;
-        entries_[k].dict_matches = DictTracker::kDeadM;
-      }
-      touch_all_ = true;
-      predicted_death_ = fc_death;
-    }
-  };
-  if (nseg > 1 && warmup_bytes_ > 0) {
-    Warmup(0, false, which, rbuf, nullptr);
-    timeline().stamp("warmed-up");
-    forecast(0, nseg);
-    tm.stop(&stats_.ms_warmup);
-  }
-  if (!allow_restart && !saved_block_guess_.empty()) {
-    for (uint32_t k = 0; k < nseg; ++k) {
-      if (!(segments_[k].flags & kSegFirstInBlock)) continue;
-      auto it = saved_block_guess_.find(segments_[k].blk_start);
-      if (it == saved_block_guess_.end()) continue;
-      memcpy(entries_[k].cache, it->second.cache, sizeof(entries_[k].cache));
-      entries_[k].ext_allowed = it->second.ext_allowed;
-      touch_all_ = true;
-    }
   }
   SegGeometry geo{};
   geo.prefix_bytes = P_.prefix_bytes;
@@ -1990,12 +1920,75 @@
   bool full_round = true;
   uint32_t last_death_seg = 0xffffffffu;
   auto stamp = [&](const char* what) { timeline().stamp(what); };
+  dev_d2d(B_.flags[which ^ 1], B_.flags[which], (size_t)P_.total_bytes + 64);
+  bool flags_copied = true;
+  if (const char* w = getenv("BROTLI_MI355X_WARMUP")) warmup_bytes_ = (uint32_t)atoi(w);
+  uint64_t fc_L = 0, fc_M = 0;
+  uint32_t fc_death = nseg;
+  bool fc_found = false;
+  auto forecast = [&](uint32_t from, uint32_t upto) {
+    if (!(P_.use_dictionary && warm_lookups_.size() == nseg)) return;
+    for (uint32_t k = from; k < upto && !fc_found; ++k) {
+      fc_L += warm_lookups_[k];
+      fc_M += warm_matches_[k];
+      if (warmup_dictionary_dies(fc_L, fc_M, warmup_bytes_, segment_bytes_)) {
+        fc_death = k;
+        fc_found = true;
+      }
+    }
+    if (upto == nseg || fc_found) {
+      for (uint32_t k = fc_death + 1; k < nseg; ++k) {
+        entries_[k].dict_lookups = DictTracker::kDeadL;
+        entries_[k].dict_matches = DictTracker::kDeadM;
+      }
+      touch_all_ = true;
+      predicted_death_ = fc_death;
+    }
+  };
+  static const bool host_warmup = getenv("BROTLI_MI355X_HOST_WARMUP") != nullptr;
+  static const bool no_spree_guess = getenv("BROTLI_MI355X_NO_SPREE_GUESS") != nullptr;
+  const bool warm = nseg > 1 && warmup_bytes_ > 0;
+  bool entries_on_device = warm && !host_warmup && (allow_restart || saved_block_guess_.empty());
+  DevBlocks warm_mem;
+  WarmupBuffers WB{};
+  std::vector<SegEntry> warm_entries_dev;
+  WarmupJob warm_check;
+  if (entries_on_device) {
+    const uint32_t dry = nseg - 1, tiles = (dry + kWarmupTile - 1) / kWarmupTile;
+    WarmupShape shape{nseg, warmup_bytes_, segment_bytes_, no_spree_guess ? 0u : 1u};
+    WB.segs = warm_mem.uninit<Segment>((size_t)dry * sizeof(Segment) + 64);
+    WB.entries = warm_mem.uninit<SegEntry>((size_t)dry * sizeof(SegEntry) + 64);
+    WB.exits = warm_mem.zeroed<SegExit>((size_t)dry * sizeof(SegExit) + 64);
+    WB.tile_ops = warm_mem.uninit<WarmupOp>((size_t)tiles * 2 * sizeof(WarmupOp) + 64);
+    WB.fc_death = warm_mem.zeroed<uint32_t>(64);
+    lz77_warmup_prepare(P_, B_, shape, WB, entries_[0].cache);
+    lz77_parse_custom(P_, B_, which, rbuf, WB.segs, WB.entries, WB.exits, dry);
+    lz77_warmup_compose(P_, B_, shape, WB);
+    timeline().stamp("warm-up queued");
+    if (!selftest) stats_.segments_parsed += (uint64_t)dry * warmup_bytes_ / segment_bytes_;
+    touch_all_ = true;
+  } else if (warm) {
+    Warmup(0, false, which, rbuf, nullptr);
+    timeline().stamp("warmed-up");
+    forecast(0, nseg);
+    tm.stop(&stats_.ms_warmup);
+  }
+  if (!allow_restart && !saved_block_guess_.empty()) {
+    for (uint32_t k = 0; k < nseg; ++k) {
+      if (!(segments_[k].flags & kSegFirstInBlock)) continue;
+      auto it = saved_block_guess_.find(segments_[k].blk_start);
+      if (it == saved_block_guess_.end()) continue;
+      memcpy(entries_[k].cache, it->second.cache, sizeof(entries_[k].cache));
+      entries_[k].ext_allowed = it->second.ext_allowed;
+      touch_all_ = true;
+    }
+  }
   for (uint32_t round = 0; round < max_rounds && !done; ++round) {
     stats_.rounds++;
     stamp("| round");
     tm.stop(&stats_.ms_resolve);
     if (full_round) {
-      dev_h2d(B_.entries, entries_.data(), (size_t)nseg * sizeof(SegEntry));
+      if (!entries_on_device) dev_h2d(B_.entries, entries_.data(), (size_t)nseg * sizeof(SegEntry));
     } else {
       const uint32_t n_up = count + (uint32_t)also_upload.size();
       for (uint32_t i = 0; i < n_up; ++i) {
@@ -2052,7 +2045,8 @@
       dev_sync();
       stamp("burst-done");
     } else {
-    dev_d2d(B_.flags[which ^ 1], B_.flags[which], (size_t)P_.total_bytes + 64);
+    if (!flags_copied) dev_d2d(B_.flags[which ^ 1], B_.flags[which], (size_t)P_.total_bytes + 64);
+    flags_copied = false;
     stamp("uploaded");
     if (full_round) {
       lz77_parse_round(P_, B_, which, rbuf, 0);
@@ -2088,6 +2082,15 @@
     if (full_round) {
       dev_d2h_async(exits_.data(), B_.exits, (size_t)nseg * sizeof(SegExit));
       touch_all_ = true;
+      if (entries_on_device) {
+        if (selftest) {
+          warm_entries_dev.resize(nseg);
+          WarmupPlan(&warm_check, 0, nseg, false, nullptr);
+          dev_d2h_async(warm_check.wexits.data(), WB.exits, (size_t)(nseg - 1) * sizeof(SegExit));
+        }
+        dev_d2h_async(selftest ? warm_entries_dev.data() : entries_.data(), B_.entries, (size_t)nseg * sizeof(SegEntry));
+        dev_d2h_async(&warm_fc_death_, WB.fc_death, 4);
+      }
     } else {
       lz77_gather_results(B_, list_dev, count, dirty_dev, nseg, got_exits_dev, cont_count_dev, cont_index_dev, cont_exits_dev, cont_entries_dev);
       dev_d2h_async(got_exits, got_exits_dev, (size_t)count * sizeof(SegExit));
@@ -2112,6 +2115,29 @@
     }
     }
     const uint32_t n_changed = counts[0], n_cont = counts[1];
+    if (entries_on_device) {
+      entries_on_device = false;
+      if (selftest) {
+        warm_check.launched = false;
+        WarmupEnd(&warm_check);
+        forecast(0, nseg);
+        static_assert(sizeof(SegEntry) == 64, "16 words");
+        for (uint32_t k = 0; k < nseg; ++k) {
+          uint32_t host_words[16], dev_words[16];
+          memcpy(host_words, &entries_[k], 64);
+          memcpy(dev_words, &warm_entries_dev[k], 64);
+          for (uint32_t w = 0; w < 16; ++w)
+            if (host_words[w] != dev_words[w])
+              throw std::runtime_error("selftest: entry composed on the device differs from the host's (segment " + std::to_string(k) + ", word " +
+                                       std::to_string(w) + ": " + std::to_string(dev_words[w]) + " vs " + std::to_string(host_words[w]) + ")");
+        }
+        if (fc_death != warm_fc_death_)
+          throw std::runtime_error("selftest: forecast of the dictionary's death differs (device segment " + std::to_string(warm_fc_death_) +
+                                   ", host " + std::to_string(fc_death) + ")");
+      }
+      if (P_.use_dictionary) predicted_death_ = warm_fc_death_;
+      warm_mem.clear();
+    }
     if (!full_round && !burst) {
       for (uint32_t i = 0; i < count; ++i) {
         exits_[list[i]] = got_exits[i];
diff --git a/rust-brotli_amd/csrc/lz77_stage.h b/rust-brotli_amd/csrc/lz77_stage.h
--- a/rust-brotli_amd/csrc/lz77_stage.h
+++ b/rust-brotli_amd/csrc/lz77_stage.h
@@ -136,8 +136,10 @@
     DevBlocks mem;
     uint32_t count = 0;
     bool dict_dead = false, whole_input = true;
+    bool launched = true;
     int mark = 0;
   };
+  uint32_t WarmupPlan(WarmupJob* job, uint32_t first_seg, uint32_t end_seg, bool dict_dead, const std::vector<uint8_t>* only_after_dirty);
   void Warmup(uint32_t first_seg, bool dict_dead, int which, int rbuf, const std::vector<uint8_t>* only_after_dirty);
   void WarmupBegin(WarmupJob* job, uint32_t first_seg, uint32_t end_seg, bool dict_dead, int which, int rbuf,
                    const std::vector<uint8_t>* only_after_dirty, int mark);
@@ -182,7 +184,8 @@
   std::vector<uint32_t> block_first_segment_, block_segment_bytes_;
   std::vector<uint8_t> coarse_blocks_;
   uint32_t total_cmd_slots_ = 0;
-  std::vector<double> warm_lookups_, warm_matches_;
+  std::vector<uint64_t> warm_lookups_, warm_matches_;
+  uint32_t warm_fc_death_ = 0;
   uint32_t predicted_death_ = 0xffffffffu;
   int final_flags_ = 0;
   const StreamCarry* carry_ = nullptr;
diff --git a/rust-brotli_amd/csrc/lz77_warmup.h b/rust-brotli_amd/csrc/lz77_warmup.h
--- /dev/null
+++ b/rust-brotli_amd/csrc/lz77_warmup.h
@@ -0,0 +1,166 @@
+#ifndef BROTLI_MI355X_LZ77_WARMUP_H_
+#define BROTLI_MI355X_LZ77_WARMUP_H_
+
+#include <math.h>
+#include <stdint.h>
+
+#include "lz77_types.h"
+
+#if defined(__HIPCC__)
+#define BR_HD __host__ __device__ inline
+#else
+#define BR_HD inline
+#endif
+
+namespace brotli_mi355x {
+
+static constexpr uint32_t kWarmDeadL = 0x40000000u, kWarmDeadM = 0, kWarmAliveL = 0, kWarmAliveM = 0x01000000u;
+static constexpr uint32_t kWarmupTile = 256;
+
+struct WarmupShape {
+  uint32_t num_segments;
+  uint32_t warmup_bytes;
+  uint32_t segment_bytes;
+  uint32_t spree_guess;
+};
+
+BR_HD Segment warmup_segment(Segment g, uint32_t warmup_bytes) {
+  if (g.end - g.start > warmup_bytes) g.start = g.end - warmup_bytes;
+  g.flags = (g.flags & kSegTailStitched) | kSegWarmup;
+  return g;
+}
+BR_HD SegEntry warmup_entry(SegEntry e, const Segment& dry, uint32_t spree_window, bool dict_dead) {
+  e.pos = dry.start;
+  e.apply = dry.start + spree_window;
+  e.dict_lookups = dict_dead ? kWarmDeadL : kWarmAliveL;
+  e.dict_matches = dict_dead ? kWarmDeadM : kWarmAliveM;
+  return e;
+}
+
+struct WarmupOp {
+  uint32_t np;
+  int32_t d[4];
+  uint64_t sl, sm;
+};
+BR_HD WarmupOp warmup_identity() {
+  WarmupOp o;
+  o.np = 0;
+  o.d[0] = o.d[1] = o.d[2] = o.d[3] = 0;
+  o.sl = o.sm = 0;
+  return o;
+}
+BR_HD WarmupOp warmup_op(const Segment& seg, const SegExit& x, uint32_t entered_lookups, uint32_t entered_matches, uint32_t warmup_bytes) {
+  WarmupOp o;
+  o.np = x.n_pushes < 4 ? x.n_pushes : 4;
+  for (uint32_t c = 0; c < 4; ++c) o.d[c] = c < o.np ? x.cache[c] : 0;
+  const uint32_t len = seg.end - seg.start;
+  const uint64_t weight = len <= warmup_bytes ? warmup_bytes : len;
+  o.sl = (uint64_t)(x.dict_lookups - entered_lookups) * weight;
+  o.sm = (uint64_t)(x.dict_matches - entered_matches) * weight;
+  return o;
+}
+BR_HD WarmupOp warmup_combine(const WarmupOp& a, const WarmupOp& b) {
+  WarmupOp o;
+  o.np = a.np + b.np < 4 ? a.np + b.np : 4;
+  for (uint32_t c = 0; c < 4; ++c) o.d[c] = c < b.np ? b.d[c] : (c - b.np < a.np ? a.d[c - b.np] : 0);
+  o.sl = a.sl + b.sl;
+  o.sm = a.sm + b.sm;
+  return o;
+}
+BR_HD void warmup_apply_cache(const WarmupOp& o, const int32_t base[4], int32_t out[4]) {
+  int32_t r[4];
+  for (uint32_t c = 0; c < 4; ++c) r[c] = c < o.np ? o.d[c] : base[c - o.np];
+  for (uint32_t c = 0; c < 4; ++c) out[c] = r[c];
+}
+
+BR_HD bool warmup_dictionary_dies(uint64_t sl, uint64_t sm, uint32_t warmup_bytes, uint32_t segment_bytes) {
+  const double sample = (double)warmup_bytes / (double)segment_bytes;
+  const double L = (double)sl / (double)warmup_bytes, M = (double)sm / (double)warmup_bytes;
+  const double ms = M * sample;
+  const double sigma = sqrt(ms > 1.0 ? ms : 1.0) / sample;
+  return L >= 256.0 && M + 3.0 * sigma < L / 128.0;
+}
+
+BR_HD void warmup_entry_from_exit(const Segment& seg, const Segment& next, const SegExit& x, uint32_t max_backward_limit, SegEntry* e) {
+  if (!(next.flags & kSegFirstInBlock)) {
+    e->pos = x.pos;
+    e->apply = x.apply;
+    e->head_kind = x.tail_kind;
+    e->head_base = x.tail_base;
+    e->head_p1 = x.tail_p1;
+  } else {
+    e->ext_allowed = 0;
+    if (x.n_cmds > 0 && x.insert_len == 0 && x.pos >= seg.blk_end) {
+      const uint64_t cmd_dist = (uint64_t)(int64_t)x.cache[0];
+      if (x.last_dist_code < 16 || (uint64_t)x.last_dist_code - 15 == cmd_dist) {
+        const uint64_t lpp = (uint64_t)next.blk_start - x.last_copy_len;
+        if (cmd_dist <= (lpp < max_backward_limit ? lpp : (uint64_t)max_backward_limit)) e->ext_allowed = 1;
+      }
+    }
+  }
+}
+
+BR_HD void warmup_predict_literal_run(uint32_t htl_, uint32_t spree_window, const Segment& seg, const SegEntry& e, SegExit* x) {
+  const uint64_t pos_end = seg.blk_end, htl = htl_, window = spree_window;
+  const uint64_t margin = htl - 1 > 4 ? htl - 1 : 4;
+  uint64_t position = e.pos;
+  const uint64_t apply = e.apply;
+  uint32_t tail_kind = e.head_kind;
+  uint64_t tail_base = e.head_base;
+  uint64_t stop = pos_end > htl ? pos_end - htl : 0;
+  if (seg.end < stop) stop = seg.end;
+  if (position < stop && position < apply) position = stop < apply ? stop : apply;
+  const uint64_t block_tail = pos_end > margin + 16 ? pos_end - margin - 16 : 0;
+  for (uint32_t pass = 0; pass < 2; ++pass) {
+    const uint64_t step = pass == 0 ? 9 : 17;
+    const uint64_t p_limit = pass == 0 ? apply + 4 * window : ~0ull >> 1;
+    if (!(position < stop)) break;
+    if (pass == 1 && !(position + 1 > apply + 4 * window)) break;
+    uint64_t bound = stop;
+    const uint64_t bt = block_tail > 0 ? block_tail - 1 : 0;
+    if (bt < bound) bound = bt;
+    if (p_limit < bound) bound = p_limit;
+    if (position >= bound) continue;
+    const uint64_t n = (bound - position + step - 1) / step;
+    tail_kind = pass == 0 ? (uint32_t)kHeadEven4 : (uint32_t)kHeadVec4;
+    tail_base = position + (n - 1) * step + 1;
+    position += n * step;
+  }
+  if (position < stop && position + 1 >= block_tail && position + 1 > apply) {
+    tail_kind = kHeadUnstored;
+    tail_base = position + 1;
+    position = pos_end;
+  }
+  if (seg.flags & kSegLastInBlock) position = pos_end;
+  x->pos = (uint32_t)position;
+  x->apply = (uint32_t)apply;
+  x->insert_len = (uint32_t)position - e.pos;
+  x->tail_kind = position > seg.end ? tail_kind : (uint32_t)kHeadNone;
+  x->tail_base = position > seg.end ? (uint32_t)tail_base : 0u;
+  x->tail_p1 = position > seg.end ? e.head_p1 : 0u;
+}
+
+BR_HD bool warmup_spree_carries(const Segment& seg, const Segment& next, const SegEntry& e, const SegExit& x) {
+  if (x.n_cmds != 0) return false;
+  if (next.flags & kSegFirstInBlock) return false;
+  if ((seg.flags & kSegFirstInBlock) && e.ext_allowed) return false;
+  return true;
+}
+BR_HD void warmup_spree_step(uint32_t htl, uint32_t spree_window, const Segment& seg, SegEntry from, SegEntry* e) {
+  if (seg.flags & kSegFirstInBlock) {
+    from.pos = seg.blk_start;
+    from.apply = from.pos + spree_window;
+    from.head_kind = kHeadNone;
+    from.head_base = from.head_p1 = 0;
+  }
+  SegExit x;
+  warmup_predict_literal_run(htl, spree_window, seg, from, &x);
+  e->pos = x.pos;
+  e->apply = x.apply;
+  e->head_kind = x.tail_kind;
+  e->head_base = x.tail_base;
+  e->head_p1 = x.tail_p1;
+}
+
+}
+#endif
diff --git a/rust-brotli_amd/csrc/lz77_warmup_emu.inc b/rust-brotli_amd/csrc/lz77_warmup_emu.inc
--- /dev/null
+++ b/rust-brotli_amd/csrc/lz77_warmup_emu.inc
@@ -0,0 +1,74 @@
+
+namespace brotli_mi355x {
+
+void lz77_warmup_prepare(const Lz77Params& P, const Lz77Buffers& B, const WarmupShape& S, const WarmupBuffers& W, const int32_t base_cache[4]) {
+  for (uint32_t k = 0; k < S.num_segments; ++k) {
+    if (k == 0) W.fc_death[0] = S.num_segments;
+    const Segment g = B.segments[k];
+    SegEntry e{};
+    e.pos = g.start;
+    e.apply = g.start + P.spree_window;
+    for (int c = 0; c < 4; ++c) e.cache[c] = base_cache[c];
+    if (k != 0) {
+      e.dict_lookups = kWarmAliveL;
+      e.dict_matches = kWarmAliveM;
+    }
+    B.entries[k] = e;
+    if (k + 1 < S.num_segments) {
+      const Segment dry = warmup_segment(g, S.warmup_bytes);
+      W.segs[k] = dry;
+      W.entries[k] = warmup_entry(e, dry, P.spree_window, false);
+    }
+  }
+}
+
+void lz77_warmup_compose(const Lz77Params& P, const Lz77Buffers& B, const WarmupShape& S, const WarmupBuffers& W) {
+  if (S.num_segments < 2) return;
+  const uint32_t count = S.num_segments - 1;
+  const uint32_t tiles = (count + kWarmupTile - 1) / kWarmupTile;
+  auto op_of = [&](uint32_t i) { return warmup_op(B.segments[i], W.exits[i], W.entries[i].dict_lookups, W.entries[i].dict_matches, S.warmup_bytes); };
+  for (uint32_t tile = 0; tile < tiles; ++tile) {
+    WarmupOp acc = warmup_identity();
+    for (uint32_t i = tile * kWarmupTile; i < count && i < (tile + 1) * kWarmupTile; ++i) acc = warmup_combine(acc, op_of(i));
+    W.tile_ops[tile] = acc;
+  }
+  WarmupOp carry = warmup_identity();
+  for (uint32_t tile = 0; tile < tiles; ++tile) {
+    W.tile_ops[tiles + tile] = carry;
+    carry = warmup_combine(carry, W.tile_ops[tile]);
+  }
+  for (uint32_t tile = 0; tile < tiles; ++tile) {
+    WarmupOp upto = W.tile_ops[tiles + tile];
+    for (uint32_t i = tile * kWarmupTile; i < count && i < (tile + 1) * kWarmupTile; ++i) {
+      upto = warmup_combine(upto, op_of(i));
+      SegEntry e = B.entries[i + 1];
+      warmup_apply_cache(upto, B.entries[0].cache, e.cache);
+      warmup_entry_from_exit(B.segments[i], B.segments[i + 1], W.exits[i], P.max_backward_limit, &e);
+      B.entries[i + 1] = e;
+      if (P.use_dictionary && warmup_dictionary_dies(upto.sl, upto.sm, S.warmup_bytes, S.segment_bytes) && i < W.fc_death[0]) W.fc_death[0] = i;
+    }
+  }
+  auto carries = [&](uint32_t j) { return warmup_spree_carries(B.segments[j], B.segments[j + 1], B.entries[j], W.exits[j]); };
+  for (uint32_t k = 0; k < S.num_segments; ++k) {
+    if (P.use_dictionary && k > W.fc_death[0]) {
+      B.entries[k].dict_lookups = kWarmDeadL;
+      B.entries[k].dict_matches = kWarmDeadM;
+    }
+  }
+  for (uint32_t k = 0; k < count && S.spree_guess; ++k) {
+    if (!carries(k) || (k > 0 && carries(k - 1))) continue;
+    SegEntry cur = B.entries[k];
+    for (uint32_t j = k; j < count && (j == k || carries(j)); ++j) {
+      SegEntry next{};
+      warmup_spree_step(P.htl, P.spree_window, B.segments[j], cur, &next);
+      B.entries[j + 1].pos = next.pos;
+      B.entries[j + 1].apply = next.apply;
+      B.entries[j + 1].head_kind = next.head_kind;
+      B.entries[j + 1].head_base = next.head_base;
+      B.entries[j + 1].head_p1 = next.head_p1;
+      cur = next;
+    }
+  }
+}
+
+}
```

Result: faster. 4730 MB/s, median of 6 (+5.9%).
